# nackdai/aten

Hardware: AMD Instinct MI355X
Metric: Mrays/sec (W*H*spp/1e6/s, reference definition), Sponza 1080p 1spp 5-bounce (higher is better)
Workload: dtype f32; 1 GPU; sponza_lod 1920x1080 1spp 5-bounce GGX+IBL, reference-built sponza_lod.sbvh (stand-in for missing sponza.obj); width=1920, height=1080, spp=1, max_depth=5, rr_depth=3, frames_in_flight=4, triangles=12852, bvh_nodes=38000, anyhit_twins=1, planar_area_lights=0

## Files before the change

### aten_amd/_lib.py

```python
import ctypes as C
import os

from . import build

_lib = None

K_NAMES = ["gen_path", "trace_closest", "shade", "trace_shadow", "accumulate_sample", "gather",
           "svgf_prepare", "svgf_temporal", "svgf_variance", "svgf_atrous", "trace_fused"]

SYMBOLS = [
    "atn_create", "atn_destroy", "atn_last_error", "atn_upload_scene", "atn_update_camera", "atn_update_tlas",
    "atn_init_sampler", "atn_set_random", "atn_set_screen_shard", "atn_render", "atn_reset", "atn_set_path_batches",
    "atn_set_frames_in_flight", "atn_bank_streams", "atn_side_stream", "atn_mgpu_set_frames_in_flight", "atn_set_sampling_options", "atn_sample_texture",
    "atn_svgf_render", "atn_svgf_set_motion_depth", "atn_svgf_reset", "atn_svgf_set_atrous_iterations",
    "atn_svgf_download", "atn_svgf_output_device", "atn_svgf_set_dilate_temporal_weight", "atn_svgf_denoise", "atn_svgf_upload",
    "atn_restir_set_options", "atn_restir_render", "atn_restir_set_motion_depth", "atn_restir_reset", "atn_restir_capture",
    "atn_restir_download", "atn_npr_render", "atn_npr_reset", "atn_npr_capture", "atn_npr_download",
    "atn_volume_render", "atn_volume_reset", "atn_volume_capture", "atn_volume_download", "atn_volume_phase_table",
    "atn_ao_set_params", "atn_ao_render", "atn_ao_reset", "atn_ao_capture", "atn_ao_download",
    "atn_film_device", "atn_tile_device", "atn_tile_slots", "atn_anyhit_twins", "atn_planar_area_lights", "atn_stream", "atn_synchronize",
    "atn_assemble_tiles", "atn_assemble_tiles_on", "atn_download_film", "atn_upload_film", "atn_get_stats", "atn_get_kernel_times",
    "atn_reset_kernel_times", "atn_generate_paths", "atn_trace_closest", "atn_cmj_samples", "atn_cmj_batch", "atn_ray_offset", "atn_get_random", "atn_random_count",
    "atn_material_table", "atn_material_eval", "atn_compact", "atn_compact2", "atn_sizeof_scene_desc", "atn_sizeof_destination",
    "atn_abi_version", "atn_build_id",
    "atn_download_path_cost", "atn_update_geometry", "atn_scene_device_arrays", "atn_lbvh_rebuild_list", "atn_lbvh_build",
    "atn_mgpu_update_geometry", "atn_mgpu_lbvh_rebuild_list",
    "atn_skin_create", "atn_skin_update", "atn_skin_compute", "atn_lbvh_rebuild_list_skinned", "atn_skin_download",
    "atn_skin_download_list", "atn_skin_destroy",
    "atn_set_geometry_motion", "atn_geometry_motion_stats", "atn_geometry_motion_matrices",
    "atn_taa_resolve", "atn_taa_upload", "atn_taa_download", "atn_taa_reset", "atn_taa_output_device", "atn_taa_rgba8_device",
    "atn_mgpu_create", "atn_mgpu_destroy", "atn_mgpu_last_error", "atn_mgpu_shard_count", "atn_mgpu_shard_device",
    "atn_mgpu_upload_scene", "atn_mgpu_update_tlas", "atn_mgpu_update_camera", "atn_mgpu_init_sampler",
    "atn_mgpu_set_random", "atn_mgpu_render", "atn_mgpu_reset", "atn_mgpu_synchronize", "atn_mgpu_film_device",
    "atn_mgpu_download_film",
    "atn_set_regeneration", "atn_get_regeneration", "atn_render_burst", "atn_regen_stage_counts",
    "atn_mgpu_set_regeneration", "atn_mgpu_render_burst", "atn_set_upload_options", "atn_libm_probe", "atn_set_shade_math",
]


class Destination(C.Structure):
    _fields_ = [("width", C.c_int32), ("height", C.c_int32), ("maxDepth", C.c_int32),
                ("russianRouletteDepth", C.c_int32), ("sample", C.c_int32), ("frame", C.c_uint32),
                ("progressive", C.c_int32), ("break_on_terminate", C.c_int32),
                ("count_stats", C.c_int32), ("profile", C.c_int32)]


def lib():
    global _lib
    if _lib is None:
        path = os.environ.get("ATEN_AMD_LIB", build.HIP_LIB)
        if not os.path.exists(path):
            raise RuntimeError(
                "aten_amd: %s is missing. Build it with `python -m aten_amd.build hip` "
                "(or __graft_entry__.build()); there is no CPU fallback." % path)
        l = C.CDLL(path)
        vp = C.c_void_p
        l.atn_create.argtypes = [C.POINTER(vp), C.c_int]
        l.atn_destroy.argtypes = [vp]; l.atn_destroy.restype = None
        l.atn_last_error.argtypes = [vp]; l.atn_last_error.restype = C.c_char_p
        l.atn_upload_scene.argtypes = [vp, vp]
        l.atn_update_camera.argtypes = [vp, vp]
        l.atn_update_tlas.argtypes = [vp, vp, C.c_uint32, vp, C.c_uint32, vp, C.c_uint32]
        l.atn_download_path_cost.argtypes = [vp, vp]
        l.atn_update_geometry.argtypes = [vp, vp, vp, C.c_uint32, C.c_uint32, vp, C.c_uint32, C.c_uint32]
        l.atn_scene_device_arrays.argtypes = [vp, vp, vp, vp]
        l.atn_lbvh_rebuild_list.argtypes = [vp, C.c_uint32, C.c_uint32, C.c_uint32, vp, vp]
        l.atn_lbvh_build.argtypes = [vp, vp, C.c_uint32, C.c_int32, vp, vp, vp, C.c_uint32, C.c_int32, vp, vp, vp]
        l.atn_skin_create.argtypes = [vp, vp, C.c_uint32, C.c_uint32, C.c_uint32, C.c_uint32, C.c_uint32, C.POINTER(C.c_uint32)]
        l.atn_skin_update.argtypes = [vp, C.c_uint32, vp, C.c_uint32]
        l.atn_skin_compute.argtypes = [vp, C.c_uint32, C.c_int32, vp, vp]
        l.atn_lbvh_rebuild_list_skinned.argtypes = [vp, C.c_uint32, C.c_uint32]
        l.atn_skin_download.argtypes = [vp, C.c_uint32, C.c_int32, vp]
        l.atn_skin_download_list.argtypes = [vp, C.c_uint32, vp, C.c_uint32, C.POINTER(C.c_uint32)]
        l.atn_skin_destroy.argtypes = [vp, C.c_uint32]
        l.atn_set_geometry_motion.argtypes = [vp, C.c_int32]
        l.atn_geometry_motion_stats.argtypes = [vp, vp]
        l.atn_geometry_motion_matrices.argtypes = [vp, vp, vp]
        l.atn_mgpu_update_geometry.argtypes = [vp, vp, vp, C.c_uint32, C.c_uint32, vp, C.c_uint32, C.c_uint32]
        l.atn_mgpu_lbvh_rebuild_list.argtypes = [vp, C.c_uint32, C.c_uint32, C.c_uint32, vp, vp]
        l.atn_init_sampler.argtypes = [vp, C.c_int32, C.c_int32, C.c_int32]
        l.atn_set_random.argtypes = [vp, vp, C.c_uint32]
        l.atn_get_random.argtypes = [vp, vp, C.c_uint32]
        l.atn_random_count.argtypes = [vp]; l.atn_random_count.restype = C.c_uint32
        l.atn_set_screen_shard.argtypes = [vp, C.c_int32, C.c_int32]
        l.atn_render.argtypes = [vp, C.POINTER(Destination), vp]
        l.atn_reset.argtypes = [vp]
        l.atn_set_upload_options.argtypes = [vp, C.c_int32, C.c_int32, C.c_int32, C.c_int32]
        l.atn_set_regeneration.argtypes = [vp, C.c_int32]
        l.atn_set_shade_math.argtypes = [vp, C.c_int32]
        l.atn_get_regeneration.argtypes = [vp]; l.atn_get_regeneration.restype = C.c_int32
        l.atn_render_burst.argtypes = [vp, C.POINTER(Destination), C.c_int32, vp]
        l.atn_regen_stage_counts.argtypes = [vp, vp, vp, C.c_uint32, C.POINTER(C.c_uint32)]
        l.atn_set_path_batches.argtypes = [vp, C.c_int32]
        l.atn_set_frames_in_flight.argtypes = [vp, C.c_int32]
        l.atn_bank_streams.argtypes = [vp, C.POINTER(C.c_int32), C.POINTER(C.c_int32)]
        l.atn_set_sampling_options.argtypes = [vp, C.c_int32, C.c_int32]
        l.atn_sample_texture.argtypes = [vp, C.c_int32, C.c_uint32, vp, vp]
        l.atn_mgpu_set_frames_in_flight.argtypes = [vp, C.c_int32]
        l.atn_svgf_render.argtypes = [vp, vp, C.c_int32, vp, vp]
        l.atn_svgf_set_motion_depth.argtypes = [vp, vp, C.c_uint32]
        l.atn_svgf_reset.argtypes = [vp]
        l.atn_svgf_set_atrous_iterations.argtypes = [vp, C.c_int32]
        l.atn_svgf_download.argtypes = [vp, C.c_int32, vp]
        l.atn_restir_set_options.argtypes = [vp, C.c_int32, C.c_int32]
        l.atn_restir_render.argtypes = [vp, vp, C.c_int32, vp]
        l.atn_restir_set_motion_depth.argtypes = [vp, vp, C.c_uint32]
        l.atn_restir_reset.argtypes = [vp]
        l.atn_restir_capture.argtypes = [vp, C.c_int32]
        l.atn_restir_download.argtypes = [vp, C.c_int32, vp]
        l.atn_npr_render.argtypes = [vp, vp, vp]
        l.atn_npr_reset.argtypes = [vp]
        l.atn_npr_capture.argtypes = [vp, C.c_int32]
        l.atn_npr_download.argtypes = [vp, C.c_int32, vp]
        l.atn_volume_render.argtypes = [vp, vp, vp]
        l.atn_volume_reset.argtypes = [vp]
        l.atn_volume_capture.argtypes = [vp, C.c_int32]
        l.atn_volume_download.argtypes = [vp, C.c_int32, vp]
        l.atn_volume_phase_table.argtypes = [vp, C.c_float, C.c_uint32, vp, vp, vp, vp, vp, vp]
        l.atn_ao_set_params.argtypes = [vp, C.c_int32, C.c_float, C.c_int32]
        l.atn_ao_render.argtypes = [vp, vp, vp]
        l.atn_ao_reset.argtypes = [vp]
        l.atn_ao_capture.argtypes = [vp, C.c_int32]
        l.atn_ao_download.argtypes = [vp, C.c_int32, vp]
        l.atn_svgf_set_dilate_temporal_weight.argtypes = [vp, C.c_int32]
        l.atn_svgf_denoise.argtypes = [vp, vp, C.c_int32, vp, vp]
        l.atn_svgf_upload.argtypes = [vp, C.c_int32, C.c_int32, C.c_int32, vp]
        l.atn_svgf_output_device.argtypes = [vp]
        l.atn_svgf_output_device.restype = vp
        l.atn_taa_resolve.argtypes = [vp, C.c_int32, C.c_int32, C.c_int32, C.c_int32, C.c_float, vp, vp]
        l.atn_taa_upload.argtypes = [vp, C.c_int32, C.c_int32, C.c_int32, vp]
        l.atn_taa_download.argtypes = [vp, C.c_int32, vp]
        l.atn_taa_reset.argtypes = [vp]
        l.atn_taa_output_device.argtypes = [vp]; l.atn_taa_output_device.restype = vp
        l.atn_taa_rgba8_device.argtypes = [vp]; l.atn_taa_rgba8_device.restype = vp
        l.atn_film_device.argtypes = [vp]; l.atn_film_device.restype = vp
        l.atn_tile_device.argtypes = [vp]; l.atn_tile_device.restype = vp
        l.atn_tile_slots.argtypes = [vp]; l.atn_tile_slots.restype = C.c_uint32
        l.atn_anyhit_twins.argtypes = [vp]; l.atn_anyhit_twins.restype = C.c_uint32
        l.atn_planar_area_lights.argtypes = [vp]; l.atn_planar_area_lights.restype = C.c_uint32
        l.atn_stream.argtypes = [vp]; l.atn_stream.restype = vp
        l.atn_side_stream.argtypes = [vp]; l.atn_side_stream.restype = vp
        l.atn_synchronize.argtypes = [vp]
        l.atn_assemble_tiles.argtypes = [vp, vp, C.c_int32, vp]
        l.atn_assemble_tiles_on.argtypes = [vp, vp, C.c_int32, vp, vp]
        l.atn_download_film.argtypes = [vp, vp]
        l.atn_upload_film.argtypes = [vp, C.c_int32, C.c_int32, vp]
        l.atn_get_stats.argtypes = [vp, vp]
        l.atn_get_kernel_times.argtypes = [vp, vp, vp]
        l.atn_reset_kernel_times.argtypes = [vp]
        l.atn_generate_paths.argtypes = [vp, C.c_int32, C.c_int32, C.c_int32, C.c_uint32, vp]
        l.atn_trace_closest.argtypes = [vp, vp, C.c_uint32, C.c_float, C.c_float, vp, vp]
        l.atn_cmj_samples.argtypes = [vp, C.c_uint32, C.c_uint32, C.c_uint32, C.c_int32, vp]
        l.atn_cmj_batch.argtypes = [vp, C.c_uint32, vp, vp, vp, C.c_int32, vp]
        l.atn_ray_offset.argtypes = [vp, C.c_uint32, vp, vp, vp]
        l.atn_libm_probe.argtypes = [vp, C.c_int32, C.c_uint32, vp, vp, vp]
        l.atn_material_table.argtypes = [vp, C.c_int32, C.c_uint32, vp, vp, vp, vp, vp, vp, vp, vp]
        l.atn_material_eval.argtypes = [vp, C.c_int32, C.c_uint32, vp, vp, vp, vp, vp]
        l.atn_compact.argtypes = [vp, vp, C.c_uint32, vp, C.POINTER(C.c_uint32)]
        l.atn_compact2.argtypes = [vp, vp, vp, C.c_uint32, C.c_uint32, vp, C.POINTER(C.c_uint32), vp, C.POINTER(C.c_uint32)]
        l.atn_mgpu_create.argtypes = [C.POINTER(vp), vp, C.c_int32]
        l.atn_mgpu_destroy.argtypes = [vp]; l.atn_mgpu_destroy.restype = None
        l.atn_mgpu_last_error.argtypes = [vp]; l.atn_mgpu_last_error.restype = C.c_char_p
        l.atn_mgpu_shard_count.argtypes = [vp]; l.atn_mgpu_shard_count.restype = C.c_int32
        l.atn_mgpu_shard_device.argtypes = [vp, C.c_int32]; l.atn_mgpu_shard_device.restype = C.c_int32
        l.atn_mgpu_upload_scene.argtypes = [vp, vp]
        l.atn_mgpu_update_tlas.argtypes = [vp, vp, C.c_uint32, vp, C.c_uint32, vp, C.c_uint32]
        l.atn_mgpu_update_camera.argtypes = [vp, vp]
        l.atn_mgpu_init_sampler.argtypes = [vp, C.c_int32, C.c_int32, C.c_int32]
        l.atn_mgpu_set_random.argtypes = [vp, vp, C.c_uint32]
        l.atn_mgpu_render.argtypes = [vp, C.POINTER(Destination), vp]
        l.atn_mgpu_reset.argtypes = [vp]
        l.atn_mgpu_set_regeneration.argtypes = [vp, C.c_int32]
# ... 10 lines not shown
```

### aten_amd/csrc/aten_amd.hip

```cpp
#include <hip/hip_runtime.h>

#include <algorithm>
#include <cstdio>
#include <cstdlib>
#include <chrono>
#include <cstring>
#include <memory>
#include <random>
#include <string>
#include <vector>

#include "../../include/aten_amd.h"
#include "device/kernels.hpp"
#include "device/launch.hpp"
#include "device/svgf.hpp"
#include "device/restir.hpp"
#include "device/npr.hpp"
#include "device/ao.hpp"
#include "device/volume.hpp"
#include "device/lbvh.hpp"
#include "device/skinning.hpp"
#include "device/motion.hpp"
#include "device/taa.hpp"
#include "host/scene_upload.hpp"
#include "host/ibl_precompute.hpp"

namespace atn {

#define ATN_HIP(expr)                                                                      \
    do {                                                                                   \
        hipError_t e_ = (expr);                                                            \
        if (e_ != hipSuccess) { return fail(ATN_ERR_HIP, std::string(#expr) + ": " + hipGetErrorString(e_)); } \
    } while (0)

template <class T>
struct DevBuf {
    T* p = nullptr;
    size_t n = 0;
    ~DevBuf() { release(); }
    void release() { if (p) { (void)hipFree(p); p = nullptr; n = 0; } }
    hipError_t resize(size_t count)
    {
        if (count <= n && p) return hipSuccess;
        release();
        if (count == 0) return hipSuccess;
        hipError_t e = hipMalloc((void**)&p, count * sizeof(T) + 256);
        if (e == hipSuccess) n = count;
        return e;
    }
    void swap(DevBuf& o) { std::swap(p, o.p); std::swap(n, o.n); }
    hipError_t upload(const std::vector<T>& v, hipStream_t s)
    {
        hipError_t e = resize(v.size() ? v.size() : 1);
        if (e != hipSuccess || v.empty()) return e;
        return hipMemcpyAsync(p, v.data(), v.size() * sizeof(T), hipMemcpyHostToDevice, s);
    }
};

__global__ void k_spin(unsigned long long ticks)
{
    const unsigned long long t0 = wall_clock64();
    while (wall_clock64() - t0 < ticks) { }
}
constexpr unsigned long long kSpinTicks = 30000;
inline bool streams_run_side_by_side(hipStream_t a, hipStream_t b, bool& ok)
{
    const double spin_us = (double)kSpinTicks / 100.0;
    for (int rep = 0; rep < 3; rep++) {
        if (hipStreamSynchronize(a) != hipSuccess || hipStreamSynchronize(b) != hipSuccess) { ok = false; return false; }
        const auto t0 = std::chrono::steady_clock::now();
        hipLaunchKernelGGL(k_spin, dim3(1), dim3(1), 0, a, kSpinTicks);
        hipLaunchKernelGGL(k_spin, dim3(1), dim3(1), 0, b, kSpinTicks);
        if (hipStreamSynchronize(a) != hipSuccess || hipStreamSynchronize(b) != hipSuccess) { ok = false; return false; }
        const double us = std::chrono::duration<double, std::micro>(std::chrono::steady_clock::now() - t0).count();
        ok = true;
        if (us < 1.5 * spin_us) return true;
    }
    ok = true;
    return false;
}

class PathTracing {
public:
    std::string last_error;
    int device = 0;
    hipStream_t stream = nullptr;
    static constexpr int kMaxBatches = 8;
    static constexpr int kMaxShards = 64;
    hipStream_t bstream[kMaxBatches] = {};
    hipEvent_t ev_fork = nullptr, ev_join[kMaxBatches] = {};
    int n_batches = 3;
    bool batches_forced = false;
    bool fuse_traces = true;
    bool env_probe_streams = true;
    bool env_lds_nodes = true;
    int env_anyhit_twin = 1;
    int env_anyhit_twin_dirs = 8;
    bool opt_node_layout = true, opt_planar_lights = true;
    bool env_atrous4 = true;
    int env_shade_waves = 0;
    int env_flavour = -1;

    DevBuf<float4> nodes, vtx_pos, vtx_nml, matrices, texels, carpaint, shade_tris;
    DevBuf<atn_triangle_param> tris;
    DevBuf<atn_object_param> objects;
    DevBuf<DevMaterial> materials;
    DevBuf<atn_light_param> lights;
    DevBuf<float4> light_plane;
    DevBuf<DevTexture> textures;
    DevBuf<atn_toon_param> toon;
    DevBuf<atn_light_param> npr_lights;
    DevBuf<float> screen_shadow;
    DevBuf<uint32_t> texels8;
    DevScene scene{};
    bool has_scene = false, has_camera = false;
    std::vector<int32_t> list_root_link;
    uint32_t n_planar_lights = 0;
    struct PlanarCert {
        int32_t inst_obj = -1, mesh_obj = -1, mtx_id = -1;
        atn_object_param inst{}, mesh{};
        atn_mat4 l2w{}, w2l{};
        uint32_t tri_first = 0, tri_count = 0, vtx_lo = 0, vtx_hi = 0;
    };
    std::vector<PlanarCert> planar_certs;
    void collect_planar_certs(const atn_scene_desc* s, const std::vector<atn_light_param>& lights)
    {
        planar_certs.clear();
        for (size_t i = 0; i < lights.size() && i < s->n_lights; i++) {
            if (!lights[i]._pad) continue;
            PlanarCert c;
            c.inst_obj = s->lights[i].arealight_objid;
            c.inst = s->objects[c.inst_obj];
            const atn_object_param* o = &s->objects[c.inst_obj];
            if (o->type == ATN_OBJ_INSTANCE) {
                c.mtx_id = o->mtx_id;
                if (c.mtx_id >= 0) { c.l2w = s->matrices[c.mtx_id]; c.w2l = s->matrices[c.mtx_id + 1]; }
                c.mesh_obj = o->object_id;
                c.mesh = s->objects[c.mesh_obj];
                o = &s->objects[c.mesh_obj];
            }
            c.tri_first = (uint32_t)o->triangle_id; c.tri_count = (uint32_t)o->triangle_num;
            c.vtx_lo = 0xFFFFFFFFu; c.vtx_hi = 0;
            for (uint32_t t = c.tri_first; t < c.tri_first + c.tri_count; t++)
                for (int k = 0; k < 3; k++) {
                    const uint32_t v = (uint32_t)s->triangles[t].idx[k];
                    c.vtx_lo = std::min(c.vtx_lo, v); c.vtx_hi = std::max(c.vtx_hi, v);
                }
            planar_certs.push_back(c);
        }
    }
    bool planar_certs_survive_objects(const atn_object_param* objs, uint32_t n_objs, const atn_mat4* mtxs, uint32_t n_mtxs) const
    {
        for (const PlanarCert& c : planar_certs) {
            if ((uint32_t)c.inst_obj >= n_objs || std::memcmp(&objs[c.inst_obj], &c.inst, sizeof(atn_object_param)) != 0) return false;
            if (c.mesh_obj >= 0 && ((uint32_t)c.mesh_obj >= n_objs || std::memcmp(&objs[c.mesh_obj], &c.mesh, sizeof(atn_object_param)) != 0)) return false;
            if (c.mtx_id >= 0 && n_mtxs
                && ((uint32_t)c.mtx_id + 1 >= n_mtxs || std::memcmp(&mtxs[c.mtx_id], &c.l2w, sizeof(atn_mat4)) != 0
                    || std::memcmp(&mtxs[c.mtx_id + 1], &c.w2l, sizeof(atn_mat4)) != 0)) return false;
        }
        return true;
    }
    bool planar_certs_survive_geometry(uint32_t vtx_offset, uint32_t n_vtx, uint32_t tri_offset, uint32_t n_tr) const
    {
        for (const PlanarCert& c : planar_certs) {
            if (n_vtx && vtx_offset <= c.vtx_hi && (uint64_t)vtx_offset + n_vtx > c.vtx_lo) return false;
            if (n_tr && tri_offset < c.tri_first + c.tri_count && (uint64_t)tri_offset + n_tr > c.tri_first) return false;
        }
        return true;
    }
    std::vector<int32_t> list_twin_delta;
    std::vector<HostSceneImage::TlasRef> tlas_refs;
    uint32_t top_base = 0, n_host_matrices = 0;
    std::vector<atn_mat4> host_matrices;
    std::vector<uint32_t> list_base, list_bytes, list_tri_leaves, list_inner;
    uint32_t n_scene_tris = 0, n_scene_vtx = 0, n_scene_mtrls = 0;

    struct LbvhScratch {
        DevBuf<uint32_t> codes[2], indices[2], counts, totals, arrived, offs;
        DevBuf<uint8_t> flips;
        DevBuf<int32_t> left, right, parent, first, last;
        DevBuf<atn_bvh_node> ref_nodes;
        DevBuf<LbvhBox> pre, suf, sup;
        DevBuf<atn_triangle_param> tris;
// ... 393 lines not shown
        t->tick = cur_tick;
        cur_tick = ++tick_counter;
        point_scene_at_current_set();
        return ATN_OK;
    }

    hipEvent_t ev_scene = nullptr, ev_stage = nullptr;
    hipStream_t scene_stream = nullptr;
    hipStream_t upd = nullptr;
    uint64_t scene_epoch = 0, bank_epoch = 0;
    bool stage_busy = false;
    char* stage_p = nullptr;
    size_t stage_cap = 0, stage_used = 0;

    int begin_scene_update(size_t stage_bytes)
    {
        if (!ev_scene) { ATN_HIP(hipEventCreateWithFlags(&ev_scene, hipEventDisableTiming)); ATN_HIP(hipEventCreateWithFlags(&ev_stage, hipEventDisableTiming)); }
        if (stage_busy) { ATN_HIP(hipEventSynchronize(ev_stage)); stage_busy = false; }
        stage_used = 0;
        if (stage_bytes > stage_cap) {
            if (stage_p) ATN_HIP(hipHostFree(stage_p));
            stage_p = nullptr; stage_cap = 0;
            const size_t cap = stage_bytes + stage_bytes / 2 + 4096;
            ATN_HIP(hipHostMalloc((void**)&stage_p, cap, hipHostMallocDefault));
            stage_cap = cap;
        }
        if (frames_in_flight > 1 && !scene_stream) ATN_HIP(hipStreamCreateWithFlags(&scene_stream, hipStreamNonBlocking));
        upd = frames_in_flight > 1 ? scene_stream : stream;
        if (frames_in_flight > 1 && n_spare_ready > 0 && !scene_in_place) {
            if (frame_since_update) { int r = flip_scene_set(); if (r) return r; frame_since_update = false; }
            return ATN_OK;
        }
        if (n_alt > 0 && frames_in_flight <= 1) drop_alt_set();
        log_now.clear();
        if (upd != stream) {
            for (int i = 0; i < n_spare_ready; i++) if (spare[i].ev_gather) ATN_HIP(hipStreamWaitEvent(upd, spare[i].ev_gather, 0));
            if (ev_gather) ATN_HIP(hipStreamWaitEvent(upd, ev_gather, 0));
        }
        return ATN_OK;
    }
    int stage_copy(void* dst_dev, const void* src_host, size_t bytes)
    {
        if (!bytes) return ATN_OK;
        const size_t off = (stage_used + 63) & ~(size_t)63;
        if (off + bytes > stage_cap) return fail(ATN_ERR_INVALID_ARG, "staging arena too small (internal)");
        std::memcpy(stage_p + off, src_host, bytes);
        stage_used = off + bytes;
        ATN_HIP(hipMemcpyAsync(dst_dev, stage_p + off, bytes, hipMemcpyHostToDevice, upd));
        return ATN_OK;
    }
    int end_scene_update()
    {
        if (stage_used) { ATN_HIP(hipEventRecord(ev_stage, upd)); stage_busy = true; }
        ATN_HIP(hipEventRecord(ev_scene, upd));
        scene_epoch++;
        if (upd == stream) bank_epoch = scene_epoch;
        return ATN_OK;
    }
    int record_scene_read()
    {
        ATN_HIP(hipEventRecord(ev_gather, stream));
        hipEvent_t& e = ev_read[bank_scene_set];
        if (!e) ATN_HIP(hipEventCreateWithFlags(&e, hipEventDisableTiming));
        ATN_HIP(hipEventRecord(e, stream));
        return ATN_OK;
    }
    int wait_scene_epoch()
    {
        if (bank_epoch != scene_epoch && ev_scene) ATN_HIP(hipStreamWaitEvent(stream, ev_scene, 0));
        bank_epoch = scene_epoch;
        bank_scene_set = cur_set;
        frame_since_update = true;
        return ATN_OK;
    }

    float k_ms[ATN_K_COUNT] = {};
    uint32_t k_launches[ATN_K_COUNT] = {};
    std::vector<hipEvent_t> ev_pool;
    struct Span { int kind; size_t e0, e1; };
    static constexpr size_t kMaxSpans = 8192;
    std::vector<Span> spans;
    size_t ev_used = 0;
    hipStream_t prof_stream = nullptr;
    uint64_t host_stats[8] = {};

    int fail(int code, const std::string& msg) { last_error = msg; return code; }

    int init(int device_ordinal)
    {
        int n = 0;
        hipError_t e = hipGetDeviceCount(&n);
        if (e != hipSuccess || n <= 0) return fail(ATN_ERR_NO_DEVICE, "no HIP device available (libaten_amd has no CPU fallback)");
        if (device_ordinal < 0 || device_ordinal >= n) return fail(ATN_ERR_INVALID_ARG, "device ordinal out of range");
        device = device_ordinal;
        ATN_HIP(hipSetDevice(device));
        ATN_HIP(hipStreamCreateWithFlags(&stream, hipStreamNonBlocking));
        for (int k = 0; k < kMaxBatches; k++) {
            ATN_HIP(hipStreamCreateWithFlags(&bstream[k], hipStreamNonBlocking));
            ATN_HIP(hipEventCreateWithFlags(&ev_join[k], hipEventDisableTiming));
        }
        ATN_HIP(hipEventCreateWithFlags(&ev_fork, hipEventDisableTiming));
        ATN_HIP(hipEventCreateWithFlags(&ev_gather, hipEventDisableTiming));
        if (const char* e = std::getenv("ATEN_AMD_FUSE")) fuse_traces = e[0] != '0';
        if (const char* e = std::getenv("ATEN_AMD_SVGF_ATROUS4")) env_atrous4 = e[0] != '0';
        if (const char* e = std::getenv("ATEN_AMD_SHADE_WAVES")) { const int v = std::atoi(e); if (v == 4 || v == 5) env_shade_waves = v; }
        if (const char* e = std::getenv("ATEN_AMD_LDS_NODES")) env_lds_nodes = std::atoi(e) != 0;
        if (const char* e = std::getenv("ATEN_AMD_ANYHIT_TWIN")) env_anyhit_twin = std::max(0, std::min(2, std::atoi(e)));
        if (const char* e = std::getenv("ATEN_AMD_ANYHIT_TWIN_DIRS")) env_anyhit_twin_dirs = std::atoi(e) == 1 ? 1 : 8;
        if (const char* e = std::getenv("ATEN_AMD_NODE_LAYOUT")) opt_node_layout = std::atoi(e) != 0;
        if (const char* e = std::getenv("ATEN_AMD_PLANAR_LIGHTS")) opt_planar_lights = std::atoi(e) != 0;
        if (const char* e = std::getenv("ATEN_AMD_PROBE_STREAMS")) env_probe_streams = std::atoi(e) != 0;
        if (const char* e = std::getenv("ATEN_AMD_TRACE")) { env_flavour = e[0] == 'r' ? 1 : 0; }
        if (const char* e = std::getenv("ATEN_AMD_BATCHES")) {
            n_batches = std::atoi(e);
            batches_forced = true;
            if (n_batches < 1) n_batches = 1;
            if (n_batches > kMaxBatches) n_batches = kMaxBatches;
        }
        return ATN_OK;
    }

    ~PathTracing()
    {
        for (auto& e : ev_pool) (void)hipEventDestroy(e);
        for (int k = 0; k < kMaxBatches; k++) {
            if (ev_join[k]) (void)hipEventDestroy(ev_join[k]);
            if (bstream[k]) (void)hipStreamDestroy(bstream[k]);
        }
        if (ev_fork) (void)hipEventDestroy(ev_fork);
        if (rs_ev) (void)hipEventDestroy(rs_ev);
        if (ta_ev) (void)hipEventDestroy(ta_ev);
        if (gm_ev) (void)hipEventDestroy(gm_ev);
        if (ao_ev) (void)hipEventDestroy(ao_ev);
        if (ev_gather) (void)hipEventDestroy(ev_gather);
        for (auto& e : sv_ev_prepare) if (e) (void)hipEventDestroy(e);
        if (ev_film) (void)hipEventDestroy(ev_film);
        if (sv_stream) (void)hipStreamDestroy(sv_stream);
        for (int i = 0; i < n_spare_ready; i++) {
            Bank& b = spare[i];
            for (int k = 0; k < kMaxBatches; k++) {
                if (b.ev_join[k]) (void)hipEventDestroy(b.ev_join[k]);
                if (b.bstream[k]) (void)hipStreamDestroy(b.bstream[k]);
            }
            if (b.ev_fork) (void)hipEventDestroy(b.ev_fork);
            if (b.ev_gather) (void)hipEventDestroy(b.ev_gather);
            for (auto& e : b.ev_read) if (e) (void)hipEventDestroy(e);
            if (b.stream) (void)hipStreamDestroy(b.stream);
        }
        if (stream) (void)hipStreamDestroy(stream);
        if (side_stream) (void)hipStreamDestroy(side_stream);
        if (scene_stream) (void)hipStreamDestroy(scene_stream);
        for (auto& e : ev_read) if (e) (void)hipEventDestroy(e);
        if (ev_scene) (void)hipEventDestroy(ev_scene);
        if (ev_stage) (void)hipEventDestroy(ev_stage);
        if (stage_p) (void)hipHostFree(stage_p);
    }

    int UpdateSceneData(const atn_scene_desc* s)
    {
        ATN_HIP(hipSetDevice(device));
        { int q = quiesce(); if (q) return q; }
        drop_alt_set(); cur_set = 0; scene_in_place = false; frame_since_update = true;
        skins.clear();
        HostSceneImage img;
        std::string err;
        const int layout_top = opt_node_layout ? kLayoutTopLevels : 0;
        const bool planar_lights = opt_planar_lights;
        if (!build_host_image(img, s, err, env_anyhit_twin, env_anyhit_twin_dirs, layout_top, planar_lights)) return fail(ATN_ERR_UNSUPPORTED, err);
        n_planar_lights = 0;
        for (const atn_light_param& l : img.lights) n_planar_lights += l._pad != 0 ? 1u : 0u;
        collect_planar_certs(s, img.lights);
        ATN_HIP(nodes.upload(img.nodes, stream));
        ATN_HIP(tris.upload(img.tris, stream));
        ATN_HIP(vtx_pos.upload(img.vtx_pos, stream));
        ATN_HIP(vtx_nml.upload(img.vtx_nml, stream));
        ATN_HIP(objects.upload(img.objects, stream));
        ATN_HIP(matrices.upload(img.matrices, stream));
        ATN_HIP(materials.upload(img.materials, stream));
        ATN_HIP(carpaint.upload(img.carpaint, stream));
        ATN_HIP(toon.upload(img.toon, stream));
        ATN_HIP(npr_lights.upload(img.npr_lights, stream));
        ATN_HIP(screen_shadow.upload(img.screen_shadow, stream));
        ATN_HIP(lights.upload(img.lights, stream));
        ATN_HIP(light_plane.upload(img.light_plane, stream));
        ATN_HIP(texels.upload(img.texels, stream));
        ATN_HIP(texels8.upload(img.texels8, stream));
        ATN_HIP(textures.upload(img.textures, stream));
        ATN_HIP(shade_tris.resize((size_t)kShadeTriQuads * (img.tris.size() ? img.tris.size() : 1)));
        if (!img.tris.empty())
// ... 472 lines not shown
    {
        if (!has_scene) return fail(ATN_ERR_NO_SCENE, "atn_upload_scene has not been called");
        if (list == 0 || list >= list_base.size()) return fail(ATN_ERR_INVALID_ARG, "not a bottom-level BVH list");
        const int32_t twin_word = list < list_twin_delta.size() ? list_twin_delta[list] : 0;
        const uint32_t twin_delta = (uint32_t)(twin_word & ~15), twin_dirs = twin_word == 0 ? 0u : ((twin_word & 1) ? 8u : 1u);
        const uint64_t bytes = twin_dirs ? (uint64_t)twin_delta * (1u + twin_dirs) : list_bytes[list];
        if ((uint64_t)list_base[list] + bytes > nodes.n * sizeof(float4)) return fail(ATN_ERR_UNSUPPORTED, "the list's region leaves the node image (internal)");
        if (n_bytes) *n_bytes = (uint32_t)bytes;
        if (!out) return ATN_OK;
        if (capacity < bytes) return fail(ATN_ERR_INVALID_ARG, "output buffer too small for the list");
        ATN_HIP(hipSetDevice(device));
        { int q = quiesce(); if (q) return q; }
        ATN_HIP(hipMemcpyAsync(out, reinterpret_cast<char*>(nodes.p) + list_base[list], bytes, hipMemcpyDeviceToHost, stream));
        ATN_HIP(hipStreamSynchronize(stream));
        return ATN_OK;
    }

    int updateCamera(const atn_camera_param* c)
    {
        if (!c) return fail(ATN_ERR_INVALID_ARG, "null camera");
        camera = *c;
        has_camera = true;
        return ATN_OK;
    }

    int setRandom(const uint32_t* v, uint32_t n)
    {
        if (!v || n == 0) return fail(ATN_ERR_INVALID_ARG, "empty seed array");
        ATN_HIP(hipSetDevice(device));
        { int q = quiesce(); if (q) return q; }
        ATN_HIP(seeds.resize(n));
        ATN_HIP(hipMemcpyAsync(seeds.p, v, (size_t)n * 4, hipMemcpyHostToDevice, stream));
        ATN_HIP(hipStreamSynchronize(stream));
        n_seeds = n;
        return ATN_OK;
    }

    int getRandom(uint32_t* out, uint32_t n)
    {
        if (!out || n == 0 || n > n_seeds) return fail(ATN_ERR_INVALID_ARG, "atn_get_random: null output or more entries than the sampler holds");
        ATN_HIP(hipSetDevice(device));
        { int q = quiesce(); if (q) return q; }
        ATN_HIP(hipMemcpyAsync(out, seeds.p, (size_t)n * 4, hipMemcpyDeviceToHost, stream));
        ATN_HIP(hipStreamSynchronize(stream));
        return ATN_OK;
    }

    int initSampler(int32_t w, int32_t h, int32_t seed)
    {
        if (w <= 0 || h <= 0) return fail(ATN_ERR_INVALID_ARG, "bad sampler size");
        std::vector<uint32_t> v((size_t)w * h);
        std::mt19937 src(seed);
        for (auto& x : v) x = (uint32_t)src();
        return setRandom(v.data(), (uint32_t)v.size());
    }

    int ensure_frame(int32_t w, int32_t h, int32_t max_depth)
    {
        const int32_t tx = (w + 7) / 8, ty = (h + 7) / 8;
        const uint32_t n_tiles = (uint32_t)tx * ty;
        const uint32_t tiles_per_rank = (n_tiles + world - 1) / world;
        const uint32_t slots = tiles_per_rank * 64;
        if (slots > kShadowSlotMask) return fail(ATN_ERR_UNSUPPORTED, "more than 2^26 path slots per GPU (shard the screen)");
        if (slots != n_slots) {
            ATN_HIP(ray_o.resize(slots)); ATN_HIP(ray_d.resize(slots)); ATN_HIP(thr.resize(slots));
            ATN_HIP(contrib.resize(slots)); ATN_HIP(isect.resize(slots));
            ATN_HIP(sh_o.resize(slots)); ATN_HIP(sh_d.resize(slots)); ATN_HIP(sh_c.resize(slots));
            ATN_HIP(accum.resize(slots)); ATN_HIP(done.resize(slots));
            ATN_HIP(queue0.resize(slots)); ATN_HIP(queue1.resize(slots)); ATN_HIP(shadow_q.resize(slots));
            ATN_HIP(tile_out.resize(slots));
            n_slots = slots;
        }
        if (w != film_w || h != film_h) {
            if (frames_in_flight > 1) { int qrc = quiesce(); if (qrc) return qrc; }
            ATN_HIP(film.resize((size_t)w * h));
            ATN_HIP(hipMemsetAsync(film.p, 0, (size_t)w * h * sizeof(float4), stream));
            film_w = w; film_h = h;
        }
        if (max_depth + 2 > counters_depth) {
            ATN_HIP(counters.resize((size_t)kMaxBatches * 4 * (max_depth + 2)));
            counters_depth = max_depth + 2;
        }
        if (!stats.p) {
            ATN_HIP(stats.resize(8));
            ATN_HIP(hipMemsetAsync(stats.p, 0, 64, stream));
        }
        return ATN_OK;
    }

    PathBuffers buffers(bool count, int batch = 0, uint32_t slot_begin = 0)
    {
        PathBuffers pb{};
        pb.ray_o = ray_o.p; pb.ray_d = ray_d.p; pb.thr = thr.p; pb.contrib = contrib.p; pb.seeds = seeds.p;
        pb.isect = isect.p; pb.sh_o = sh_o.p; pb.sh_d = sh_d.p; pb.sh_c = sh_c.p;
        pb.accum = accum.p; pb.done = done.p; pb.queue[0] = queue0.p + slot_begin; pb.queue[1] = queue1.p + slot_begin;
        pb.shadow_q = shadow_q.p + slot_begin;
        uint32_t* cb = counters.p + (size_t)batch * 4 * counters_depth;
        pb.q_count = cb; pb.sh_count = cb + counters_depth;
        pb.fetch_closest = cb + 2 * counters_depth; pb.fetch_shadow = cb + 3 * counters_depth;
        pb.stats = count ? stats.p : nullptr;
        pb.cost = count ? cost.p : nullptr;
        return pb;
    }

    FrameParams frame_params(const atn_destination& d)
    {
        FrameParams fp{};
        fp.width = d.width; fp.height = d.height; fp.n_slots = (int32_t)n_slots;
        fp.tiles_x = (d.width + 7) / 8; fp.tiles_y = (d.height + 7) / 8; fp.tiles_x_rcp = udiv_rcp((uint32_t)fp.tiles_x);
        fp.rank = rank; fp.world = world;
        fp.max_depth = d.maxDepth;
        fp.rr_depth = d.russianRouletteDepth;
        if (fp.rr_depth > fp.max_depth) fp.rr_depth = fp.max_depth - 1;
        fp.slot_begin = 0; fp.slot_end = (int32_t)n_slots;
        fp.chunk_items = kChunkItems;
        fp.sample = 0; fp.frame = d.frame; fp.n_seeds = n_seeds;
        fp.break_on_terminate = d.break_on_terminate; fp.progressive = d.progressive;
        return fp;
    }

    static uint32_t grid_for(uint32_t n, uint32_t cap_blocks = 256u * 16u)
    {
        uint32_t b = (n + 255u) / 256u;
        if (b == 0) b = 1;
        return b < cap_blocks ? b : cap_blocks;
    }

    bool tree_is_deep = false;
    static constexpr size_t kRefillMinNodes = 2048;
    static constexpr uint32_t kRefillMinPaths = 400u * 1000u;
    bool refill_walk(bool frame) const
    {
        if (env_flavour >= 0) return env_flavour == 1;
        return tree_is_deep && (!frame || n_slots >= kRefillMinPaths);
    }

    uint32_t lds_scene_bytes() const
    {
        const uint64_t b = (uint64_t)scene.node_bytes + (uint64_t)scene.mtx_quads * 16u;
        return (env_lds_nodes && b <= kLdsNodesMaxBytes) ? (uint32_t)b : 0u;
    }

    uint32_t trace_grid(uint32_t n_jobs, bool refill) const
    {
        if (refill) {
            const uint32_t waves_per_block = (uint32_t)kTraceBlock / 64u;
            uint32_t blocks = ((n_jobs + atn::kFetchChunk - 1u) / atn::kFetchChunk + waves_per_block - 1u) / waves_per_block;
            if (blocks < 1u) blocks = 1u;
            const uint32_t cap = (frames_in_flight > 1 ? 256u * 18u : 256u * 32u) / waves_per_block;
            return blocks < cap ? blocks : cap;
        }
        return grid_for(n_jobs);
    }

    PassPlan plan_pass(PassKind kind, uint32_t n) const
    {
        PassPlan p{};
        p.kind = kind;
        p.refill = refill_walk(true);
        p.lds_bytes = lds_scene_bytes();
        p.block = p.lds_bytes > 8192u ? 256u : 64u;
        p.trace_grid = trace_grid(n, p.refill);
        p.fused_grid = trace_grid(2u * n, p.refill);
        p.shade_items = n >= 400u * 1000u ? kChunkItems : 2;
        p.shade_grid = grid_for((n + (uint32_t)p.shade_items - 1u) / (uint32_t)p.shade_items);
        const bool big = n >= 1500u * 1000u;
        p.shade_waves = env_shade_waves ? env_shade_waves
                      : (kind == PassKind::Serial && frames_in_flight > 1 && (scene.material_set != kMsCore || big) ? 5 : 4);
        return p;
    }

    template <bool SHADOW>
    void launch_trace(const PassPlan& p, const PathBuffers& pb, bool count, int32_t b, hipStream_t st)
    {
        const dim3 g(p.trace_grid), t(p.refill ? (uint32_t)kTraceBlock : 256u);
        with_flags([&](auto c, auto refill) {
            if constexpr (SHADOW) hipLaunchKernelGGL((k_trace_shadow<decltype(c)::value, decltype(refill)::value>), g, t, 0, st, pb, scene, b);
            else hipLaunchKernelGGL((k_trace_closest<decltype(c)::value, decltype(refill)::value>), g, t, 0, st, pb, scene, b);
        }, count, p.refill);
    }

    template <bool SVGF>
    void launch_shade(const PassPlan& p, hipStream_t st, const PathBuffers& pb, const FrameParams& fp, int32_t b, const SvgfShade& sv)
    {
        if (!SVGF && shade_math_relaxed) {
            relaxed_launch_shade(scene.material_set, p.shade_waves, p.shade_grid, st, pb, scene, fp, camera, b);
            return;
        }
        with_shade_flavour(scene.material_set, p.shade_waves, [&](auto k) {
            using K = decltype(k);
            if constexpr (K::waves == 0) hipLaunchKernelGGL((k_shade<SVGF, K::ms>), dim3(p.shade_grid), dim3(256), 0, st, pb, scene, fp, camera, b, sv);
            else hipLaunchKernelGGL((k_shade_wn<SVGF, K::ms, K::waves>), dim3(p.shade_grid), dim3(256), 0, st, pb, scene, fp, camera, b, sv);
        });
    }

    void prof_begin(bool on, int kind, hipStream_t st = nullptr)
    {
        if (!st) st = stream;
        prof_stream = st;
        if (!on) return;
        if (spans.size() >= kMaxSpans) {
            (void)hipStreamSynchronize(stream);
            for (int k = 0; k < kMaxBatches; k++) (void)hipStreamSynchronize(bstream[k]);
            prof_collect();
        }
        if (ev_used + 2 > ev_pool.size()) {
            for (int i = 0; i < 64; i++) { hipEvent_t e; (void)hipEventCreate(&e); ev_pool.push_back(e); }
        }
        spans.push_back(Span{ kind, ev_used, ev_used + 1 });
        (void)hipEventRecord(ev_pool[ev_used], st);
    }
    void prof_end(bool on)
    {
        if (!on) return;
        (void)hipEventRecord(ev_pool[ev_used + 1], prof_stream);
        ev_used += 2;
    }
    void prof_collect()
    {
        for (const Span& s : spans) {
            float ms = 0;
            if (hipEventElapsedTime(&ms, ev_pool[s.e0], ev_pool[s.e1]) == hipSuccess) { k_ms[s.kind] += ms; k_launches[s.kind]++; }
        }
        spans.clear();
        ev_used = 0;
    }

    template <bool SVGF>
    int run_paths(const atn_destination* d, FrameParams fp, bool count, bool prof, const SvgfShade& sv, const SvgfFrame& sf)
    {
        int nb;
        if (batches_forced) {
            nb = n_batches;
            const uint32_t min_batch = 200u * 1000u;
            while (nb > 1 && n_slots / (uint32_t)nb < min_batch) nb--;
        }
        else {
            nb = refill_walk(true) ? 1 : (lds_scene_bytes() && frames_in_flight > 1) ? 1 : (n_slots >= (frames_in_flight > 1 ? 1500u : 800u) * 1000u ? 2 : 1);
            if (nb > n_batches) nb = n_batches;
        }
        if (nb > batch_streams_checked && nb > 1 && env_probe_streams) { int rc = separate_batch_streams(nb); if (rc) return rc; }
        uint32_t per = (n_slots + (uint32_t)nb - 1u) / (uint32_t)nb;
        per = (per + kChunk - 1u) / kChunk * kChunk;
        ATN_HIP(hipMemsetAsync(counters.p, 0, (size_t)nb * 4 * counters_depth * 4, stream));
        ATN_HIP(hipEventRecord(ev_fork, stream));
        for (int k = 0; k < nb; k++) {
            const uint32_t begin = (uint32_t)k * per;
            const uint32_t end = begin + per < n_slots ? begin + per : n_slots;
            if (begin >= end) continue;
            hipStream_t st = nb > 1 ? bstream[k] : stream;
            if (nb > 1) ATN_HIP(hipStreamWaitEvent(st, ev_fork, 0));
            PathBuffers pb = buffers(count, k, begin);
            fp.slot_begin = (int32_t)begin; fp.slot_end = (int32_t)end;
            const uint32_t n = end - begin;
            const PassPlan plan = plan_pass(SVGF ? PassKind::Svgf : PassKind::Serial, n);
            fp.chunk_items = plan.shade_items;
            const uint32_t g_slots = grid_for(n), g_all = (n + 255u) / 256u;
            for (int32_t s = 0; s < d->sample; s++) {
                fp.sample = s;
                if (s > 0) ATN_HIP(hipMemsetAsync(pb.q_count, 0, (size_t)4 * counters_depth * 4, st));
                prof_begin(prof, ATN_K_GEN, st);
                hipLaunchKernelGGL(k_gen_path, dim3(g_slots), dim3(256), 0, st, pb, fp, camera, (const uint32_t*)seeds.p);
                prof_end(prof);
                if (count || !fuse_traces) {
                    for (int32_t b = 0; b < d->maxDepth; b++) {
                        prof_begin(prof, ATN_K_TRACE_CLOSEST, st);
                        launch_trace<false>(plan, pb, count, b, st);
                        prof_end(prof);
                        if (SVGF && b == 0 && gm_capture) motion_launch_capture(g_all, st, pb, fp, gm_capture);
                        prof_begin(prof, ATN_K_SHADE, st);
                        launch_shade<SVGF>(plan, st, pb, fp, b, sv);
                        prof_end(prof);
                        prof_begin(prof, ATN_K_TRACE_SHADOW, st);
                        launch_trace<true>(plan, pb, count, b, st);
                        prof_end(prof);
                    }
                }
                else {
                    for (int32_t b = 0; b <= d->maxDepth; b++) {
                        const TraceLaunch tl = trace_launch(plan, b);
                        prof_begin(prof, tl.prof_kind, st);
                        launch_trace_fused<false>(tl, st, pb, scene, b - 1, b < d->maxDepth ? b : -1, b);
                        prof_end(prof);
                        if (SVGF && b == 0 && gm_capture) motion_launch_capture(g_all, st, pb, fp, gm_capture);
                        if (b < d->maxDepth) {
                            prof_begin(prof, ATN_K_SHADE, st);
                            launch_shade<SVGF>(plan, st, pb, fp, b, sv);
                            prof_end(prof);
                        }
                    }
                }
                if (SVGF || d->sample > 1) {
                    prof_begin(prof, ATN_K_ACCUM, st);
                    if (SVGF) hipLaunchKernelGGL(k_svgf_sample_end, dim3(g_all), dim3(256), 0, st, pb, fp, sf);
                    else hipLaunchKernelGGL(k_accumulate_sample, dim3(g_all), dim3(256), 0, st, pb, fp);
                    prof_end(prof);
                }
            }
            if (nb > 1) {
                ATN_HIP(hipEventRecord(ev_join[k], st));
                ATN_HIP(hipStreamWaitEvent(stream, ev_join[k], 0));
            }
        }
        return ATN_OK;
    }

    int check_ready(const atn_destination* d)
    {
        if (!d) return fail(ATN_ERR_INVALID_ARG, "null destination");
        if (!has_scene) return fail(ATN_ERR_NO_SCENE, "atn_upload_scene has not been called");
        if (!has_camera) return fail(ATN_ERR_INVALID_ARG, "atn_update_camera has not been called");
        if (n_seeds == 0) return fail(ATN_ERR_INVALID_ARG, "atn_init_sampler / atn_set_random has not been called");
        if (d->width <= 0 || d->height <= 0 || d->maxDepth <= 0 || d->sample <= 0) return fail(ATN_ERR_INVALID_ARG, "bad destination");
        return ATN_OK;
    }
    int begin_frame(const atn_destination& d, bool rotate)
    {
        if (rotate) swap_bank(spare[frame_seq % (uint64_t)(frames_in_flight - 1)]);
        frame_seq++;
        const int rc = wait_scene_epoch();
        return rc ? rc : ensure_frame(d.width, d.height, d.maxDepth);
    }
    int wait_film()
    {
        if (film_pending) ATN_HIP(hipStreamWaitEvent(stream, ev_film, 0));
        return taa_before_write(stream);
    }
    int record_film_writer()
    {
        if (frames_in_flight <= 1) return ATN_OK;
        if (!ev_film) ATN_HIP(hipEventCreateWithFlags(&ev_film, hipEventDisableTiming));
        ATN_HIP(hipEventRecord(ev_film, stream));
        film_pending = true;
        return ATN_OK;
    }
    int end_film_frame()
    {
        const int rc = frames_in_flight > 1 ? record_scene_read() : ATN_OK;
        return rc ? rc : record_film_writer();
    }

    int render(const atn_destination* d, atn_vec4* out_host)
    {
        int rc = check_ready(d);
        if (rc) return rc;
        ATN_HIP(hipSetDevice(device));
        if (d->sample > 1 && regen_applies(*d, 1)) return render_regen(d, 1, out_host);
        const bool count = d->count_stats != 0, prof = d->profile != 0;
        if (frames_in_flight > 1 && count) { rc = quiesce(); if (rc) return rc; }
        rc = begin_frame(*d, frames_in_flight > 1 && !count);
        if (rc) return rc;
        FrameParams fp = frame_params(*d);
        if (count) {
            ATN_HIP(hipMemsetAsync(stats.p, 0, 64, stream));
            ATN_HIP(cost.resize((size_t)2 * n_slots));
            ATN_HIP(cost_film.resize((size_t)2 * d->width * d->height));
            ATN_HIP(hipMemsetAsync(cost.p, 0, (size_t)2 * n_slots * sizeof(uint32_t), stream));
            ATN_HIP(hipMemsetAsync(cost_film.p, 0, (size_t)2 * d->width * d->height * sizeof(uint32_t), stream));
            cost_w = d->width; cost_h = d->height;
        }
        PathBuffers pb = buffers(count);

        const uint32_t g_all = (n_slots + 255u) / 256u;
        rc = run_paths<false>(d, fp, count, prof, SvgfShade{}, SvgfFrame{});
        if (rc) return rc;
        fp.slot_begin = 0; fp.slot_end = (int32_t)n_slots;
        rc = wait_film();
        if (rc) return rc;
        prof_begin(prof, ATN_K_GATHER);
        if (d->sample == 1) hipLaunchKernelGGL((k_gather<true>), dim3(g_all), dim3(256), 0, stream, pb, fp, film.p, tile_out.p);
        else hipLaunchKernelGGL((k_gather<false>), dim3(g_all), dim3(256), 0, stream, pb, fp, film.p, tile_out.p);
        prof_end(prof);
        ATN_HIP(hipGetLastError());
        rc = end_film_frame();
        if (rc) return rc;

        if (count) {
            hipLaunchKernelGGL(k_cost_to_pixels, dim3(g_all), dim3(256), 0, stream, fp, (const uint32_t*)cost.p, cost_film.p);
            ATN_HIP(hipMemcpyAsync(host_stats, stats.p, 64, hipMemcpyDeviceToHost, stream));
        }
        if (out_host) {
            ATN_HIP(hipMemcpyAsync(out_host, film.p, (size_t)d->width * d->height * sizeof(float4), hipMemcpyDeviceToHost, stream));
        }
        if (out_host || count) ATN_HIP(hipStreamSynchronize(stream));
        return ATN_OK;
    }


    bool shade_math_relaxed = false;
    int regen_mode = 0;
    uint64_t rg_host_totals[4] = {};
    static constexpr int32_t kRegenMaxStages = 1 << 16;
    static constexpr int32_t kRegenMaxDepth = 128;
    static constexpr size_t kRegenStagingBytes = (size_t)1 << 30;

    bool regen_applies(const atn_destination& d, int32_t n_frames) const
    {
        if (regen_mode == 0 || d.count_stats) return false;
        if (d.maxDepth > kRegenMaxDepth || (uint32_t)d.sample >= kRegenMaxSpp) return false;
        if ((uint64_t)n_frames * (uint64_t)d.width * (uint64_t)d.height >= kRegenMaxItems) return false;
        if (n_frames > 1 && !d.progressive) return false;
        return ((int64_t)n_frames + 1) * d.sample * d.maxDepth <= kRegenMaxStages;
    }

    int render_burst(const atn_destination* d, int32_t n_frames, atn_vec4* out_host)
    {
        if (!d) return fail(ATN_ERR_INVALID_ARG, "null destination");
        if (n_frames <= 0) return fail(ATN_ERR_INVALID_ARG, "bad burst length");
        if (regen_applies(*d, n_frames)) {
            { const int rc = check_ready(d); if (rc) return rc; }
            ATN_HIP(hipSetDevice(device));
            const uint64_t tiles = (uint64_t)((d->width + 7) / 8) * ((d->height + 7) / 8);
            const uint64_t plane = ((tiles + world - 1) / world) * 64u * sizeof(float4);
            int32_t piece = (int32_t)(kRegenStagingBytes / (plane ? plane : 1u));
            if (piece < 1) piece = 1;
            atn_destination part = *d;
            for (int32_t k = 0; k < n_frames; k += piece) {
                const int32_t n = n_frames - k < piece ? n_frames - k : piece;
                part.frame = d->frame + (uint32_t)k;
                const int rc = render_regen(&part, n, k + n == n_frames ? out_host : nullptr);
                if (rc) return rc;
            }
            return ATN_OK;
        }
        atn_destination one = *d;
        for (int32_t k = 0; k < n_frames; k++) {
            one.frame = d->frame + (uint32_t)k;
            const int rc = render(&one, k + 1 == n_frames ? out_host : nullptr);
            if (rc) return rc;
        }
        return ATN_OK;
    }

    int render_regen(const atn_destination* d, int32_t n_frames, atn_vec4* out_host)
    {
        const bool prof = d->profile != 0;
        int rc = begin_frame(*d, frames_in_flight > 1);
        if (rc) return rc;
        const int32_t stages = (n_frames + 1) * d->sample * d->maxDepth;
        rc = regen_valid_list(d->width, d->height);
        if (rc) return rc;
        if (pend.n < n_slots) ATN_HIP(pend.resize(n_slots));
        const size_t cstride = (size_t)stages + 3;
        if (rg_counters.n < 3 * cstride + 1) ATN_HIP(rg_counters.resize(3 * cstride + 1));
        if (rg_frames.n < (size_t)n_frames * n_slots) ATN_HIP(rg_frames.resize((size_t)n_frames * n_slots));
        rg_stages = stages;
        FrameParams fp = frame_params(*d);
        fp.burst_frames = n_frames; fp.spp = d->sample;
        fp.n_valid = rg_n_valid; fp.n_valid_rcp = udiv_rcp(rg_n_valid); fp.n_items = rg_n_valid * (uint32_t)n_frames;
        PathBuffers pb = buffers(false);
        pb.pend = pend.p;
        pb.valid_list = rg_valid.p; pb.next_item = rg_counters.p + 3 * cstride;
        pb.q_count = rg_counters.p + 1; pb.sh_count = rg_counters.p + cstride + 1; pb.fetch_closest = rg_counters.p + 2 * cstride + 1;
        pb.fetch_shadow = nullptr;
        const RegenOut ro{ rg_frames.p, film.p, tile_out.p };

        const uint32_t n = rg_n_valid;
        const PassPlan plan = plan_pass(PassKind::Regen, n);
        fp.chunk_items = plan.shade_items;
        const uint32_t g_all = (n_slots + 255u) / 256u;
        const uint32_t chunk_size = 256u * (uint32_t)plan.shade_items, n_chunks = (n + chunk_size - 1u) / chunk_size, n_groups = (n_chunks + kRegenGroup - 1u) / kRegenGroup;
        const size_t region_words = (size_t)n_chunks * chunk_size;
        const size_t rg_words = 2 * region_words + 2 * (size_t)n_chunks + 4 * (size_t)n_groups;
        if (rg_regions.n < rg_words) ATN_HIP(rg_regions.resize(rg_words));
        pb.q_regions = rg_regions.p; pb.sh_regions = rg_regions.p + region_words; pb.region_counts = rg_regions.p + 2 * region_words;
        uint32_t* const group_counts[2] = { pb.region_counts + 2 * (size_t)n_chunks, pb.region_counts + 2 * (size_t)n_chunks + 2 * (size_t)n_groups };

// ... 1322 lines not shown
    CTX_OR_FAIL(ctx);
    return guarded(ctx, [&] { return ctx->r.skin_update(skin, matrices, n); });
}
int atn_skin_compute(atn_ctx* ctx, atn_skin skin, int32_t is_restart, float* bbox_min, float* bbox_max)
{
    CTX_OR_FAIL(ctx);
    return guarded(ctx, [&] { return ctx->r.skin_compute(skin, is_restart != 0, bbox_min, bbox_max); });
}
int atn_lbvh_rebuild_list_skinned(atn_ctx* ctx, uint32_t list_index, atn_skin skin)
{
    CTX_OR_FAIL(ctx);
    return guarded(ctx, [&] { return ctx->r.lbvh_rebuild_list_skinned(list_index, skin); });
}
int atn_skin_download(atn_ctx* ctx, atn_skin skin, int32_t which, void* out_host)
{
    CTX_OR_FAIL(ctx);
    return guarded(ctx, [&] { return ctx->r.skin_download(skin, which, out_host); });
}
int atn_skin_download_list(atn_ctx* ctx, uint32_t list_index, void* out_host, uint32_t capacity_bytes, uint32_t* n_bytes)
{
    CTX_OR_FAIL(ctx);
    return guarded(ctx, [&] { return ctx->r.download_list(list_index, out_host, capacity_bytes, n_bytes); });
}
int atn_skin_destroy(atn_ctx* ctx, atn_skin skin)
{
    CTX_OR_FAIL(ctx);
    return guarded(ctx, [&] { return ctx->r.skin_destroy(skin); });
}
int atn_scene_device_arrays(atn_ctx* ctx, void** vtx_pos, void** vtx_nml, void** triangles)
{
    CTX_QUIET_OR_FAIL(ctx);
    if (!ctx->r.has_scene) return ctx->r.fail(ATN_ERR_NO_SCENE, "atn_upload_scene has not been called");
    { int q = ctx->r.quiesce(); if (q) return q; }
    ctx->r.drop_alt_set(); ctx->r.scene_in_place = true;
    if (ctx->r.gm_on) { const int g = ctx->r.set_geometry_motion(0); if (g) return g; }
    ctx->r.scene.planar_lights = 0;
    if (vtx_pos) *vtx_pos = ctx->r.vtx_pos.p;
    if (vtx_nml) *vtx_nml = ctx->r.vtx_nml.p;
    if (triangles) *triangles = ctx->r.tris.p;
    return ATN_OK;
}
int atn_set_geometry_motion(atn_ctx* ctx, int32_t on)
{
    CTX_QUIET_OR_FAIL(ctx);
    return guarded(ctx, [&] { return ctx->r.set_geometry_motion(on); });
}
int atn_geometry_motion_stats(atn_ctx* ctx, uint64_t* out3)
{
    CTX_OR_FAIL(ctx);
    if (!out3) return ctx->r.fail(ATN_ERR_INVALID_ARG, "null output");
    for (int k = 0; k < 3; k++) out3[k] = ctx->r.gm_stats[k];
    return ATN_OK;
}
int atn_geometry_motion_matrices(atn_ctx* ctx, float* w2c16, float* prev_w2c16)
{
    CTX_OR_FAIL(ctx);
    if (!w2c16 || !prev_w2c16) return ctx->r.fail(ATN_ERR_INVALID_ARG, "null output");
    if (!ctx->r.gm_stats[0]) return ctx->r.fail(ATN_ERR_INVALID_ARG, "no frame has been rendered with compute_motion = 2");
    std::memcpy(w2c16, ctx->r.gm_w2c, sizeof(ctx->r.gm_w2c)); std::memcpy(prev_w2c16, ctx->r.gm_prev_w2c, sizeof(ctx->r.gm_prev_w2c));
    return ATN_OK;
}
int atn_init_sampler(atn_ctx* ctx, int32_t w, int32_t h, int32_t seed) { CTX_QUIET_OR_FAIL(ctx); return guarded(ctx, [&] { return ctx->r.initSampler(w, h, seed); }); }
int atn_get_random(atn_ctx* ctx, uint32_t* out_host, uint32_t n) { CTX_QUIET_OR_FAIL(ctx); return guarded(ctx, [&] { return ctx->r.getRandom(out_host, n); }); }
uint32_t atn_random_count(atn_ctx* ctx) { return ctx ? ctx->r.n_seeds : 0; }
int atn_set_random(atn_ctx* ctx, const uint32_t* seeds, uint32_t n) { CTX_QUIET_OR_FAIL(ctx); return guarded(ctx, [&] { return ctx->r.setRandom(seeds, n); }); }

int atn_set_screen_shard(atn_ctx* ctx, int32_t rank, int32_t world)
{
    CTX_OR_FAIL(ctx);
    if (world <= 0 || rank < 0 || rank >= world) return ctx->r.fail(ATN_ERR_INVALID_ARG, "bad screen shard");
    ctx->r.rank = rank; ctx->r.world = world;
    return ATN_OK;
}

int atn_render(atn_ctx* ctx, const atn_destination* dst, atn_vec4* out_host) { CTX_OR_FAIL(ctx); return guarded(ctx, [&] { return ctx->r.render(dst, out_host); }); }
int atn_render_burst(atn_ctx* ctx, const atn_destination* dst, int32_t n_frames, atn_vec4* out_host) { CTX_OR_FAIL(ctx); return guarded(ctx, [&] { return ctx->r.render_burst(dst, n_frames, out_host); }); }
int atn_set_regeneration(atn_ctx* ctx, int32_t mode)
{
    CTX_QUIET_OR_FAIL(ctx);
    if (mode < 0 || mode > 1) return ctx->r.fail(ATN_ERR_INVALID_ARG, "regeneration mode out of range");
    ctx->r.regen_mode = mode;
    return ATN_OK;
}
int atn_set_shade_math(atn_ctx* ctx, int32_t mode)
{
    CTX_QUIET_OR_FAIL(ctx);
    if (mode < 0 || mode > 1) return ctx->r.fail(ATN_ERR_INVALID_ARG, "shade math mode out of range");
    ctx->r.shade_math_relaxed = mode == 1;
    return ATN_OK;
}
int32_t atn_get_regeneration(atn_ctx* ctx) { return ctx ? ctx->r.regen_mode : 0; }
int atn_regen_stage_counts(atn_ctx* ctx, uint32_t* closest, uint32_t* shadow, uint32_t capacity, uint32_t* n_stages)
{
    CTX_QUIET_OR_FAIL(ctx);
    return guarded(ctx, [&] { return ctx->r.regen_stage_counts(closest, shadow, capacity, n_stages); });
}
int atn_reset(atn_ctx* ctx) { CTX_QUIET_OR_FAIL(ctx); return ctx->r.reset(); }
int atn_set_path_batches(atn_ctx* ctx, int32_t n)
{
    CTX_OR_FAIL(ctx);
    if (n < 1 || n > PathTracing::kMaxBatches) return ctx->r.fail(ATN_ERR_INVALID_ARG, "batch count out of range");
    ctx->r.n_batches = n;
    ctx->r.batches_forced = n == 1;
    return ATN_OK;
}

int atn_set_sampling_options(atn_ctx* ctx, int32_t ibl_importance, int32_t tex_bilinear)
{
    CTX_OR_FAIL(ctx);
    return guarded(ctx, [&] { return ctx->r.set_sampling_options(ibl_importance, tex_bilinear); });
}

int atn_sample_texture(atn_ctx* ctx, int32_t texid, uint32_t n, const float* uv_host, float* out_host)
{
    CTX_QUIET_OR_FAIL(ctx);
    PathTracing& r = ctx->r;
    if (!r.has_scene) return r.fail(ATN_ERR_NO_SCENE, "atn_upload_scene has not been called");
    if (texid < 0 || texid >= r.scene.n_textures || n == 0 || !uv_host || !out_host) return r.fail(ATN_ERR_INVALID_ARG, "bad texture id / count");
    return guarded(ctx, [&]() -> int {
        C_HIP(r, hipSetDevice(r.device));
        atn::DevBuf<float> duv, dout;
        C_HIP(r, duv.resize(2 * (size_t)n)); C_HIP(r, dout.resize(4 * (size_t)n));
        C_HIP(r, hipMemcpyAsync(duv.p, uv_host, 8 * (size_t)n, hipMemcpyHostToDevice, r.stream));
        hipLaunchKernelGGL(atn::k_sample_texture, dim3((n + 255) / 256), dim3(256), 0, r.stream, r.scene, texid, n, (const float*)duv.p, dout.p);
        C_HIP(r, hipGetLastError());
        C_HIP(r, hipMemcpyAsync(out_host, dout.p, 16 * (size_t)n, hipMemcpyDeviceToHost, r.stream));
        C_HIP(r, hipStreamSynchronize(r.stream));
        return ATN_OK;
    });
}

int atn_set_frames_in_flight(atn_ctx* ctx, int32_t n)
{
    CTX_OR_FAIL(ctx);
    return guarded(ctx, [&] { return ctx->r.set_frames_in_flight(n); });
}

int atn_bank_streams(atn_ctx* ctx, int32_t* swaps, int32_t* concurrent)
{
    CTX_OR_FAIL(ctx);
    return guarded(ctx, [&] {
        atn::PathTracing& r = ctx->r;
        C_HIP(r, hipSetDevice(r.device));
        { int q = r.quiesce(); if (q) return q; }
        if (swaps) *swaps = r.n_stream_swaps;
        if (concurrent) {
            *concurrent = 1;
            hipStream_t st[atn::PathTracing::kMaxInFlight];
            st[0] = r.stream;
            for (int i = 1; i < r.frames_in_flight; i++) st[i] = r.spare[i - 1].stream;
            for (int i = 0; i < r.frames_in_flight; i++)
                for (int j = 0; j < i; j++) {
                    bool ok = true;
                    if (!atn::streams_run_side_by_side(st[j], st[i], ok)) *concurrent &= ~1;
                    if (!ok) return r.fail(ATN_ERR_HIP, "stream probe failed");
                }
            if (r.side_stream) {
                *concurrent |= 2;
                for (int i = 0; i < r.frames_in_flight; i++) {
                    bool ok = true;
                    if (!atn::streams_run_side_by_side(st[i], r.side_stream, ok)) *concurrent &= ~2;
                    if (!ok) return r.fail(ATN_ERR_HIP, "stream probe failed");
                }
            }
        }
        return (int)ATN_OK;
// ... 571 lines not shown
```

### aten_amd/csrc/device/kernels.hpp

```cpp
#pragma once
#include "shading.hpp"
#include "toon.hpp"

#if defined(ATN_REGEN_TU) || defined(ATN_TEMPLATES_ONLY)
#define ATN_MAIN_TU 0
#else
#define ATN_MAIN_TU 1
#endif
#ifdef ATN_REGEN_TU
#define ATN_REGEN_KERNELS 1
#else
#define ATN_REGEN_KERNELS 0
#endif

namespace atn {

constexpr uint32_t F_TERMINATED = 1u, F_SINGULAR = 2u, F_HIT = 4u;
constexpr uint32_t kShadowSlotMask = (1u << 26) - 1u;
constexpr uint32_t kShadowStencilFlag = 0x40000000u;
constexpr uint32_t F_LAST_SPECULAR = 8u;

constexpr uint32_t F_PENDING = 16u;
constexpr uint32_t kRegenFlagMask = 31u;
constexpr uint32_t kRegenBounceShift = 5u, kRegenBounceMask = 255u;
constexpr uint32_t kRegenSampleShift = 13u, kRegenSampleMask = 2047u;
constexpr uint32_t kRegenItemHiShift = 24u;
constexpr uint32_t kRegenDimMask = 4095u, kRegenItemLoShift = 12u, kRegenItemLoMask = (1u << 20) - 1u;
constexpr uint32_t kRegenMaxSpp = 1u << 11, kRegenMaxItems = 1u << 28;
constexpr uint32_t kShadowFinalFlag = 0x20000000u;

struct PathBuffers {
    float4* ray_o;
    float4* ray_d;
    float4* thr;
    float4* contrib;
    const uint32_t* seeds;
    float4* isect;
    float4* sh_o;
    float4* sh_d;
    float4* sh_c;
    float4* accum;
    uint32_t* done;
    uint32_t* queue[2];
    uint32_t* shadow_q;
    uint32_t* q_count;
    uint32_t* sh_count;
    uint32_t* fetch_closest;
    uint32_t* fetch_shadow;
    uint32_t* cost;
    unsigned long long* stats;
    float4* pend;
    uint32_t* q_regions;
    uint32_t* sh_regions;
    uint32_t* region_counts;
    uint32_t* group_counts;
    const uint32_t* valid_list;
    uint32_t* next_item;
};

struct FrameParams {
    int32_t width, height;
    int32_t n_slots;
    int32_t slot_begin, slot_end;
    int32_t chunk_items;
    int32_t tiles_x, tiles_y;
    uint32_t tiles_x_rcp;
    int32_t rank, world;
    int32_t max_depth, rr_depth;
    int32_t sample;
    uint32_t frame;
    uint32_t n_seeds;
    int32_t break_on_terminate;
    int32_t progressive;
    int32_t burst_frames, spp;
    uint32_t n_valid, n_valid_rcp, n_items;
};

ATN_DEV bool slot_to_pixel(const FrameParams& fp, uint32_t slot, int32_t& x, int32_t& y)
{
    const uint32_t local_tile = slot >> 6;
    const uint32_t in_tile = slot & 63u;
    const uint32_t tile = local_tile * (uint32_t)fp.world + (uint32_t)fp.rank;
    if (tile >= (uint32_t)(fp.tiles_x * fp.tiles_y)) return false;
    uint32_t tx, ty;
    udivmod(tile, (uint32_t)fp.tiles_x, fp.tiles_x_rcp, ty, tx);
    x = (int32_t)tx * 8 + (int32_t)(in_tile & 7u);
    y = (int32_t)ty * 8 + (int32_t)(in_tile >> 3);
    return x < fp.width && y < fp.height;
}

constexpr int kChunkItems = 4;
constexpr uint32_t kChunk = 256u * kChunkItems;

struct BlockAppendShared { uint32_t wave_total[2][4]; uint32_t base[2]; };

template <class EntryFn, bool REGION = false>
ATN_DEV void block_append2(BlockAppendShared& sh, uint32_t* qA, uint32_t* cntA, uint32_t flagsA,
                           uint32_t* qB, uint32_t* cntB, uint32_t flagsB, EntryFn entry)
{
    const uint32_t tid = here_v(threadIdx.x);
    const uint32_t lane = tid & 63u, wave = tid >> 6;
    uint32_t totA = 0, totB = 0;
#pragma unroll
    for (int k = 0; k < kChunkItems; k++) {
        totA += (uint32_t)__popcll(__ballot((flagsA >> k) & 1u));
        totB += (uint32_t)__popcll(__ballot((flagsB >> k) & 1u));
    }
    if (lane == 0) { sh.wave_total[0][wave] = totA; sh.wave_total[1][wave] = totB; }
    __syncthreads();
    if (threadIdx.x == 0) {
        const uint32_t a = sh.wave_total[0][0] + sh.wave_total[0][1] + sh.wave_total[0][2] + sh.wave_total[0][3];
        const uint32_t b = sh.wave_total[1][0] + sh.wave_total[1][1] + sh.wave_total[1][2] + sh.wave_total[1][3];
        if constexpr (REGION) { *cntA = a; *cntB = b; sh.base[0] = 0u; sh.base[1] = 0u; }
        else {
        sh.base[0] = a ? atomicAdd(cntA, a) : 0u;
        sh.base[1] = (b && cntB) ? atomicAdd(cntB, b) : 0u;
        }
    }
    __syncthreads();
    uint32_t offA = sh.base[0], offB = sh.base[1];
    for (uint32_t w = 0; w < wave; w++) { offA += sh.wave_total[0][w]; offB += sh.wave_total[1][w]; }
#pragma unroll
    for (int k = 0; k < kChunkItems; k++) {
        const unsigned long long mA = __ballot((flagsA >> k) & 1u);
        const unsigned long long mB = __ballot((flagsB >> k) & 1u);
        if ((flagsA >> k) & 1u) qA[offA + bits_below_lane(mA)] = entry(k);
        if ((flagsB >> k) & 1u) qB[offB + bits_below_lane(mB)] = entry(k);
        offA += (uint32_t)__popcll(mA);
        offB += (uint32_t)__popcll(mB);
    }
    __syncthreads();
}

ATN_DEV void wave_add_stat(unsigned long long* dst, uint32_t v)
{
    for (int off = 32; off > 0; off >>= 1) v += __shfl_down(v, off);
    if (__lane_id() == 0 && v) atomicAdd(dst, (unsigned long long)v);
}

ATN_DEV void pinhole_sample(const atn_camera_param& cam, float s, float t, f3& org, f3& dir)
// ... 140 lines not shown
__global__ void __launch_bounds__(256) k_regen_compact(PathBuffers pb, int32_t stage, uint32_t chunk_size, uint32_t* group_counts_next, uint32_t n_groups)
{
    __shared__ uint32_t red[2][4];
    const uint32_t n_prev = pb.q_count[stage - 1];
    const uint32_t n_chunks = (n_prev + chunk_size - 1u) / chunk_size;
    const uint32_t c = blockIdx.x;
    if (c == 0u) { for (uint32_t g = threadIdx.x; g < 2u * n_groups; g += 256u) group_counts_next[g] = 0u; }
    if (c >= n_chunks) return;
    const uint32_t g0 = c / kRegenGroup;
    uint32_t sq = 0, ss = 0;
    for (uint32_t g = threadIdx.x; g < g0; g += 256u) { sq += pb.group_counts[2u * g]; ss += pb.group_counts[2u * g + 1u]; }
    for (uint32_t r = g0 * kRegenGroup + threadIdx.x; r < c; r += 256u) { sq += pb.region_counts[2u * r]; ss += pb.region_counts[2u * r + 1u]; }
    for (int off = 32; off > 0; off >>= 1) { sq += __shfl_down(sq, off); ss += __shfl_down(ss, off); }
    if ((threadIdx.x & 63u) == 0u) { red[0][threadIdx.x >> 6] = sq; red[1][threadIdx.x >> 6] = ss; }
    __syncthreads();
    const uint32_t base_q = red[0][0] + red[0][1] + red[0][2] + red[0][3];
    const uint32_t base_s = red[1][0] + red[1][1] + red[1][2] + red[1][3];
    const uint32_t nq = pb.region_counts[2u * c], ns = pb.region_counts[2u * c + 1u];
    uint32_t* __restrict__ qd = pb.queue[stage & 1];
    for (uint32_t e = threadIdx.x; e < nq; e += 256u) qd[base_q + e] = pb.q_regions[(size_t)c * chunk_size + e];
    for (uint32_t e = threadIdx.x; e < ns; e += 256u) pb.shadow_q[base_s + e] = pb.sh_regions[(size_t)c * chunk_size + e];
    if (c == n_chunks - 1u && threadIdx.x == 0u) { pb.q_count[stage] = base_q + nq; pb.sh_count[stage - 1] = base_s + ns; }
}

__global__ void __launch_bounds__(256) k_regen_flush(PathBuffers pb, FrameParams fp, RegenOut ro)
{
    const uint32_t slot = blockIdx.x * blockDim.x + threadIdx.x;
    if (slot >= (fp.n_valid < fp.n_items ? fp.n_valid : fp.n_items)) return;
    const uint32_t w = __float_as_uint(pb.ray_d[slot].w);
    if (w & F_PENDING) {
        const float4 pd = pb.pend[slot];
        regen_epilogue(pb, fp, ro, slot, mk3(pd), (uint32_t)fp.spp - 1u, __float_as_uint(pd.w), true);
    }
}

__global__ void __launch_bounds__(256) k_regen_end(PathBuffers pb, FrameParams fp, RegenOut ro)
{
    const uint32_t slot = blockIdx.x * blockDim.x + threadIdx.x;
    if (slot >= (uint32_t)fp.n_slots) return;
    int32_t x, y;
    if (!slot_to_pixel(fp, slot, x, y)) {
        if (ro.tile_out) ro.tile_out[slot] = make_float4(0.0F, 0.0F, 0.0F, 0.0F);
        return;
    }
    const uint32_t pixel = (uint32_t)(y * fp.width + x);
    float4 out = make_float4(0.0F, 0.0F, 0.0F, 0.0F);
    if (fp.progressive) out = ro.film[pixel];
    for (int32_t k = 0; k < fp.burst_frames; k++) {
        const float4 v = ro.frames[(size_t)k * (uint32_t)fp.n_slots + slot];
        if (fp.progressive) {
            const float4 cur = out;
            const float n = (float)((int32_t)cur.w);
            const float d = n + 1;
            out = make_float4((n * cur.x + v.x) / d, (n * cur.y + v.y) / d, (n * cur.z + v.z) / d, n + 1);
        }
        else {
            out = v;
        }
    }
    ro.film[pixel] = out;
    if (ro.tile_out) ro.tile_out[slot] = out;
}
#endif

#ifdef ATN_TRACE_WPE
#define ATN_TRACE_ATTR __attribute__((amdgpu_waves_per_eu(ATN_TRACE_WPE, ATN_TRACE_WPE)))
#else
#define ATN_TRACE_ATTR
#endif

template <bool COUNT, bool REFILL, class Job, bool LDSN = false>
ATN_DEV void trace_dispatch(const DevScene& sc, uint32_t count, uint32_t* fetch_counter, const Job& job, TravCounters* tc)
{
    if constexpr (REFILL) {
        __shared__ TraceShared sh;
        if (LDSN) lds_scene_copy(sc);
        trace_refill<COUNT, Job, LDSN>(sc, sh, count, fetch_counter, job, tc);
    }
    else {
        trace_simple<COUNT, Job, LDSN>(sc, count, job, tc);
    }
}

struct ClosestJob {
    PathBuffers pb;
    const uint32_t* __restrict__ q;
    float t_min;
    ATN_DEV void fetch(uint32_t j, float4& a, float4& b, float& stop_t) const { fetch_slot(q[j], a, b, stop_t); }
    ATN_DEV void fetch_slot(uint32_t slot, float4& a, float4& b, float& stop_t) const
    {
        const float4 ro = pb.ray_o[slot], rd = pb.ray_d[slot];
        stop_t = -kInf;
        a = make_float4(ro.x, ro.y, ro.z, kInf);
        b = make_float4(rd.x, rd.y, rd.z, __uint_as_float(slot));
    }
    ATN_DEV bool finish(uint32_t slot, const Hit& h, bool, float4&, float4&, float&) const
    {
        pb.isect[slot] = make_float4(__int_as_float(h.objid), h.a, h.b, __int_as_float(h.tri));
        return false;
    }
    ATN_DEV void cost(uint32_t slot, uint32_t nodes, uint32_t tris) const
    {
        if (pb.cost) { atomicAdd(&pb.cost[2u * slot], nodes); atomicAdd(&pb.cost[2u * slot + 1u], tris); }
    }
};

template <bool COUNT, bool REFILL>
__global__ void __launch_bounds__(kTraceBlock > 256 ? kTraceBlock : 256) k_trace_closest(PathBuffers pb, DevScene sc, int32_t bounce)
{
    const uint32_t count = pb.q_count[bounce];
    const ClosestJob job{ pb, pb.queue[bounce & 1], kEps };
    TravCounters tc{};
    trace_dispatch<COUNT, REFILL>(sc, count, &pb.fetch_closest[bounce], job, &tc);
    if (COUNT) {
        if (blockIdx.x == 0 && threadIdx.x == 0) atomicAdd(&pb.stats[0], (unsigned long long)count);
        wave_add_stat(&pb.stats[3], tc.nodes);
        wave_add_stat(&pb.stats[4], tc.tris);
    }
}

struct SvgfShade {
    float4* nd;
    float4* am;
    float4* primary;
    float w2c3[4];
};

#ifdef ATN_SHADE_WPE
#define ATN_SHADE_ATTR __attribute__((amdgpu_waves_per_eu(ATN_SHADE_WPE, ATN_SHADE_WPE)))
#else
#define ATN_SHADE_ATTR
#endif
#ifndef ATN_SHADE_PARTITION
#define ATN_SHADE_PARTITION 1
#endif
struct ShadePartShared { uint32_t perm[kChunk]; uint32_t wcount[kChunkItems][4][2]; };
template <bool ON> struct ShadeOrderShared { uint16_t inv[ON ? kChunk : 1]; uint8_t oflag[ON ? kChunk : 1]; };

template <bool SVGF, int MS, bool REGEN = false>
ATN_DEV void shade_body(const PathBuffers& pb, const DevScene& sc, const FrameParams& fp, const atn_camera_param& cam, int32_t bounce_arg, const SvgfShade& sv,
                        const RegenOut& ro = RegenOut{})
{
    __shared__ BlockAppendShared sh;
#if ATN_SHADE_PARTITION
    __shared__ ShadePartShared part;
    __shared__ ShadeOrderShared<REGEN> order[1];
#endif
    const uint32_t count = pb.q_count[bounce_arg];
    const uint32_t* __restrict__ q = pb.queue[bounce_arg & 1];
    uint32_t* __restrict__ qn = pb.queue[(bounce_arg + 1) & 1];
#if !ATN_SHADE_PARTITION
    uint32_t nhits = 0;
#endif

    const int items = fp.chunk_items;
    const uint32_t chunk_size = 256u * (uint32_t)items;
    for (uint32_t chunk = blockIdx.x * chunk_size; chunk < count; chunk += gridDim.x * chunk_size) {
      uint32_t push_bits = 0;
#if ATN_SHADE_PARTITION
      const uint32_t n_valid = count - chunk < chunk_size ? count - chunk : chunk_size;
      {
          const uint32_t tid = here_v(threadIdx.x);
          const uint32_t lane = tid & 63u, wave = tid >> 6;
          uint32_t hitmask = 0;
          __syncthreads();
#pragma unroll 1
          for (int k = 0; k < items; k++) {
              const uint32_t j = chunk + (uint32_t)k * 256u + threadIdx.x;
              const bool valid = j < count;
              const bool hit = valid && __float_as_int(pb.isect[q[j]].x) >= 0;
              if (hit) hitmask |= 1u << k;
              const unsigned long long bh = __ballot(hit), bm = __ballot(valid && !hit);
              if (lane == 0) { part.wcount[k][wave][0] = (uint32_t)__popcll(bh); part.wcount[k][wave][1] = (uint32_t)__popcll(bm); }
          }
          if (pb.stats) wave_add_stat(&pb.stats[2], (uint32_t)__popc(hitmask));
          __syncthreads();
          uint32_t total_hits = 0;
          for (int k = 0; k < items; k++) for (uint32_t w = 0; w < 4; w++) total_hits += part.wcount[k][w][0];
          uint32_t before_h = 0, before_m = 0;
#pragma unroll 1
          for (int k = 0; k < items; k++) {
              const uint32_t j = chunk + (uint32_t)k * 256u + threadIdx.x;
              const bool valid = j < count;
              const bool hit = (hitmask >> k) & 1u;
              const unsigned long long bh = __ballot(hit), bm = __ballot(valid && !hit);
              uint32_t bh_w = before_h, bm_w = before_m;
              for (uint32_t w = 0; w < 4; w++) {
                  if (w < wave) { bh_w += part.wcount[k][w][0]; bm_w += part.wcount[k][w][1]; }
                  before_h += part.wcount[k][w][0]; before_m += part.wcount[k][w][1];
              }
              if (valid) {
                  const uint32_t pos = hit ? bh_w + bits_below_lane(bh) : total_hits + bm_w + bits_below_lane(bm);
                  part.perm[pos] = q[j];
                  if constexpr (REGEN) order[0].inv[pos] = (uint16_t)(j - chunk);
              }
          }
          __syncthreads();
      }
#endif
#pragma unroll 1
      for (int k = 0; k < items; k++) {
#if ATN_SHADE_PARTITION
        const uint32_t e = (uint32_t)k * 256u + threadIdx.x;
        const bool valid = e < n_valid;
#else
        const uint32_t j = chunk + (uint32_t)k * 256u + threadIdx.x;
        const bool valid = j < count;
#endif
        bool push_next = false, push_shadow = false;
        uint32_t rg_need_bits = 0u;
        uint32_t slot = 0;

        if (valid) {
#if ATN_SHADE_PARTITION
            slot = part.perm[e];
#else
            slot = q[j];
#endif
            const float4 ro4 = pb.ray_o[slot], rd4 = pb.ray_d[slot];
            const f3 ray_org = mk3(ro4), ray_dir = mk3(rd4);
            float pdfb = ro4.w;
            uint32_t flags = __float_as_uint(rd4.w);
            uint32_t rg_sample = 0u, rg_item = 0u;
            int32_t bounce = bounce_arg;
            if constexpr (REGEN) {
                rg_sample = (flags >> kRegenSampleShift) & kRegenSampleMask;
                rg_item = (flags >> kRegenItemHiShift) << 20;
                bounce = (int32_t)((flags >> kRegenBounceShift) & kRegenBounceMask);
                flags &= kRegenFlagMask;
            }
            const float4 is4 = pb.isect[slot];
            const int32_t hit_objid = __float_as_int(is4.x);
            const float4 thr4 = pb.thr[slot];
            f3 throughput = mk3(thr4);
            bool wrote_ray = false, thr_stored = false;
            f3 contrib_add = mk3(0.0F);
            bool contrib_changed = false;
            uint4 s4;
            uint32_t pixel_slot = slot;
            {
                uint32_t fs = fp.frame + (uint32_t)fp.sample;
                s4.y = __float_as_uint(thr4.w);
                if constexpr (REGEN) {
                    rg_item |= s4.y >> kRegenItemLoShift;
                    s4.y &= kRegenDimMask;
                    uint32_t rg_frame;
                    regen_item(pb, fp, rg_item, rg_frame, pixel_slot);
                    fs = fp.frame + rg_frame + rg_sample;
                }
                int32_t px = 0, py = 0;
                slot_to_pixel(fp, pixel_slot, px, py);
                s4.w = (uint32_t)(py * fp.width + px);
                const uint32_t rnd = pb.seeds[s4.w < fp.n_seeds ? s4.w : s4.w % here(fp.n_seeds)];
                s4.x = fs % 256u;
                s4.z = rnd * 0x1fe3434fu * ((fs + 133u * rnd) / 256u);
            }
            Cmj smp; smp.idx = s4.x; smp.dim = s4.y; smp.scramble = s4.z;
            if constexpr (REGEN) {
                if (flags & F_PENDING) {
                    flags &= ~F_PENDING;
                    const bool prev_last = rg_sample == 0u;
                    const float4 pd = pb.pend[slot];
                    regen_epilogue(pb, fp, ro, slot, mk3(pd), prev_last ? (uint32_t)fp.spp - 1u : rg_sample - 1u, __float_as_uint(pd.w), prev_last);
                }
            }
            bool rg_stored = false;
            uint32_t rg_end = 0u;
            auto regen_end = [&](bool out_of_depth) -> uint32_t {
                f3 ctot = mk3(pb.contrib[slot]);
                if (contrib_changed) ctot = ctot + contrib_add;
                const bool pending = out_of_depth;
                const bool item_last = rg_sample + 1u >= (uint32_t)fp.spp || (fp.break_on_terminate && !out_of_depth && !regen_invalid_color(ctot));
                if (pending) pb.pend[slot] = make_float4(ctot.x, ctot.y, ctot.z, __uint_as_float(rg_item));
                else regen_epilogue(pb, fp, ro, slot, ctot, rg_sample, rg_item, item_last);
                if (item_last) return pending ? 12u : 4u;
                const RegenState st = regen_primary_state(pb, fp, cam, rg_item, rg_sample + 1u, pending ? F_PENDING : 0u);
                pb.ray_o[slot] = st.o; pb.ray_d[slot] = st.d; pb.thr[slot] = st.t;
                pb.contrib[slot] = make_float4(0.0F, 0.0F, 0.0F, 0.0F);
                return 1u;
            };

            flags &= ~F_HIT;
            const bool is_hit = hit_objid >= 0;

            if (!is_hit) {
                if (!(flags & F_TERMINATED)) {
                    f3 dir = ray_dir;
                    if (bounce == 0) {
                        int32_t ix = 0, iy = 0;
                        slot_to_pixel(fp, pixel_slot, ix, iy);
                        const float s = (float)ix / (float)here(fp.width);
                        const float t = (float)iy / (float)here(fp.height);
                        f3 o;
                        pinhole_sample(cam, s, t, o, dir);
                    }
                    const float4 emit = background_sample(sc, dir);
                    float misW = 1.0f;
                    if (SVGF && (bounce == 0 || (bounce == 1 && (flags & F_SINGULAR)))) {
                        sv.nd[s4.w] = make_float4(0.0F, 0.0F, 0.0F, -1.0F);
                        sv.am[s4.w] = make_float4(emit.x, emit.y, emit.z, -1.0F);
                        if (bounce == 0) sv.primary[s4.w] = make_float4(0.0F, 0.0F, 0.0F, 0.0F);
                    }
                    if (!(bounce == 0 || (bounce == 1 && (flags & F_SINGULAR)))) {
                        float pdfLight = luminance(emit.x, emit.y, emit.z) / sc.avgIllum;
                        pdfLight /= (2.0f * kPi);
// ... 78 lines not shown
                    shaded_out = true;
                }

                if (!shaded_out) {
                    if (!(m.attrib & ATN_MTRL_ATTR_TRANSLUCENT) && isBackfacing) orienting_normal = -orienting_normal;
                    const int32_t mtrl_slot = mtrlid >= 0 ? mtrlid : sc.n_materials;
                    const float pre_r = apply_normal<MS>(sc, m, mtrl_slot, orienting_normal, rec.u, rec.v, ray_dir, smp);

                    const bool invalid_mtrl = (m.attrib & (ATN_MTRL_ATTR_SINGULAR | ATN_MTRL_ATTR_TRANSLUCENT)) != 0;
                    const bool nee = sc.n_lights > 0 && !invalid_mtrl;
                    const uint32_t nee_dim = smp.dim;
                    const f3 thr_in = throughput;
                    HitPre hp;
                    tangent_coordinate(orienting_normal, hp.t, hp.b);
                    hp.rough = ggx_roughness(sc, m, rec.u, rec.v);
                    hp.lambda_v = m.type == ATN_MTRL_GGX ? ggx_lambda(hp.rough, -ray_dir, orienting_normal) : 0.0F;
                    int32_t nee_light = 0;
                    if (nee) {
                        if (here(sc.n_lights) > 1) {
                            nee_light = (int32_t)(cmj_next(smp) * (float)here(sc.n_lights));
                            nee_light = nee_light < sc.n_lights - 1 ? nee_light : sc.n_lights - 1;
                        }
                        else smp.dim++;
                        smp.dim += light_sample_draws(sc.lights[nee_light], sc);
                    }

                    float russian_prob = 1.0f;
                    if (bounce > fp.rr_depth) {
                        if (dot(throughput, throughput) > 0) {
                            russian_prob = max3(throughput);
                            const float p = cmj_next(smp);
                            if (p >= russian_prob) flags |= F_TERMINATED; else flags &= ~F_TERMINATED;
                        }
                    }

                    MtrlSample ms;
                    sample_material<MS>(ms, sc, m, orienting_normal, ray_dir, smp, rec.u, rec.v, mtrl_slot, pre_r, &hp);
                    const f3 next_dir = normalize(ms.dir);
                    const f3 ray_along_normal = dot(orienting_normal, next_dir) >= 0.0f ? orienting_normal : -orienting_normal;
                    const float c = dot(ray_along_normal, next_dir);
                    if (ms.pdf > 0 && c > 0) {
                        throughput = throughput * ((((albedo * ms.bsdf) * c) / ms.pdf));
                        if (russian_prob != 1.0F) throughput = throughput / russian_prob;
                    }
                    else {
                        flags |= F_TERMINATED;
                    }
                    bool nee_final = false;
                    if constexpr (REGEN) {
                        bool cont = false;
                        if (!(flags & F_TERMINATED)) {
                            pdfb = ms.pdf;
                            flags = (m.attrib & ATN_MTRL_ATTR_SINGULAR) ? (flags | F_SINGULAR) : (flags & ~F_SINGULAR);
                            cont = bounce + 1 < fp.max_depth;
                            nee_final = !cont;
                        }
                        if (cont) {
                            const f3 no = ray_offset(rec.p, ray_along_normal);
                            const f3 nd = normalize(next_dir);
                            pb.ray_o[slot] = make_float4(no.x, no.y, no.z, pdfb);
                            pb.ray_d[slot] = make_float4(nd.x, nd.y, nd.z, __uint_as_float(regen_pack_d(flags, (uint32_t)(bounce + 1), rg_sample, rg_item)));
                            pb.thr[slot] = make_float4(throughput.x, throughput.y, throughput.z, __uint_as_float(regen_pack_t(smp.dim, rg_item)));
                            push_next = true;
                        }
                        else {
                            rg_end = regen_end(nee_final);
                            contrib_changed = false;
                            push_next = rg_end == 1u;
                        }
                        rg_stored = true; thr_stored = true; wrote_ray = true;
                    }
                    else {
                    pb.thr[slot] = make_float4(throughput.x, throughput.y, throughput.z, __uint_as_float(smp.dim));
                    thr_stored = true;
                    if (!(flags & F_TERMINATED)) {
                        pdfb = ms.pdf;
                        flags = (m.attrib & ATN_MTRL_ATTR_SINGULAR) ? (flags | F_SINGULAR) : (flags & ~F_SINGULAR);
                        if (SVGF) {
                            const bool last_spec = m.id >= 0 && m.id < sc.n_materials && sc.materials[m.id].type == ATN_MTRL_SPECULAR;
                            flags = last_spec ? (flags | F_LAST_SPECULAR) : (flags & ~F_LAST_SPECULAR);
                        }
                        const f3 no = ray_offset(rec.p, ray_along_normal);
                        const f3 nd = normalize(next_dir);
                        pb.ray_o[slot] = make_float4(no.x, no.y, no.z, pdfb);
                        pb.ray_d[slot] = make_float4(nd.x, nd.y, nd.z, __uint_as_float(flags));
                        wrote_ray = true;
                        push_next = (bounce + 1 < fp.max_depth);
                    }
                    }
                    if (nee && !(flags & F_TERMINATED)) {
                        Cmj sl; sl.idx = smp.idx; sl.dim = nee_dim + 1u; sl.scramble = smp.scramble;
                        const int32_t li = nee_light;
                        const float lightSelectPdf = sc.inv_n_lights;
                        LightSample ls;
                        sample_light(ls, sc.lights[li], sc, rec.p, orienting_normal, sl, &hp);
                        push_shadow = radiance_nee_then<MS>(sc, ray_dir, orienting_normal, m, rec.u, rec.v, lightSelectPdf, ls, mtrl_slot, pre_r, nullptr,
                                                            [&](const f3& radiance) {
                            const float lbits = __uint_as_float((uint32_t)li | ((m.attrib & kAttrStencilAlways) ? kShadowStencilFlag : 0u)
                                                                | (nee_final ? kShadowFinalFlag : 0u));
                            const f3 lightcontrib = (thr_in * radiance) * albedo;
                            pb.sh_c[slot] = make_float4(lightcontrib.x, lightcontrib.y, lightcontrib.z, lbits);
                            const f3 dirToLight = normalize(ls.dir);
                            const float distToLight = length(ls.pos - rec.p);
                            const f3 so = ray_offset(rec.p, orienting_normal);
                            pb.sh_o[slot] = make_float4(so.x, so.y, so.z, distToLight);
                            pb.sh_d[slot] = make_float4(dirToLight.x, dirToLight.y, dirToLight.z, lbits);
                        }, &hp);
                    }
                }
            }
            if constexpr (REGEN) {
                if (!rg_stored) {
                    rg_end = regen_end(false);
                    contrib_changed = false;
                    push_next = rg_end == 1u;
                    thr_stored = true;
                }
            }
            else if (!push_next && !wrote_ray) {
                pb.ray_d[slot] = make_float4(rd4.x, rd4.y, rd4.z, __uint_as_float(flags));
            }
            if (!thr_stored) pb.thr[slot] = make_float4(throughput.x, throughput.y, throughput.z, __uint_as_float(smp.dim));
            if (contrib_changed) {
                const f3 contrib = mk3(pb.contrib[slot]) + contrib_add;
                pb.contrib[slot] = make_float4(contrib.x, contrib.y, contrib.z, 0.0F);
            }
            if constexpr (REGEN) rg_need_bits = rg_end & 12u;
        }
        if constexpr (REGEN) {
            if (valid) order[0].oflag[order[0].inv[e]] = (uint8_t)((push_next ? 1u : 0u) | (push_shadow ? 2u : 0u) | rg_need_bits);
        }
        else push_bits |= (push_next ? 1u << k : 0u) | (push_shadow ? 0x10000u << k : 0u);
      }
#if ATN_SHADE_PARTITION
      auto entry_of = [&](int k) { return part.perm[(uint32_t)k * 256u + threadIdx.x]; };
#else
      auto entry_of = [&](int k) { return q[chunk + (uint32_t)k * 256u + threadIdx.x]; };
#endif
      if constexpr (REGEN) {
          __syncthreads();
          {
              const uint32_t tid2 = here_v(threadIdx.x);
              const uint32_t lane2 = tid2 & 63u, wave2 = tid2 >> 6;
              uint32_t tot = 0;
#pragma unroll 1
              for (int k = 0; k < items; k++) {
                  const uint32_t jl = (uint32_t)k * 256u + threadIdx.x;
                  const bool need = jl < n_valid && (order[0].oflag[jl] & 4u) != 0u;
                  tot += (uint32_t)__popcll(__ballot(need));
              }
              if (lane2 == 0u) sh.wave_total[0][wave2] = tot;
              __syncthreads();
              if (threadIdx.x == 0u) {
                  const uint32_t a = sh.wave_total[0][0] + sh.wave_total[0][1] + sh.wave_total[0][2] + sh.wave_total[0][3];
                  sh.base[0] = a ? atomicAdd(pb.next_item, a) : 0u;
              }
              __syncthreads();
              uint32_t off = sh.base[0];
              for (uint32_t w = 0; w < wave2; w++) off += sh.wave_total[0][w];
#pragma unroll 1
              for (int k = 0; k < items; k++) {
                  const uint32_t jl = (uint32_t)k * 256u + threadIdx.x;
                  uint32_t f = jl < n_valid ? (uint32_t)order[0].oflag[jl] : 0u;
                  const bool need = (f & 4u) != 0u;
                  const unsigned long long m = __ballot(need);
                  if (need) {
                      const uint32_t item = off + bits_below_lane(m);
                      const uint32_t slot2 = q[chunk + jl];
                      const uint32_t pend_flag = (f & 8u) ? F_PENDING : 0u;
                      if (item < fp.n_items) {
                          const RegenState st = regen_primary_state(pb, fp, cam, item, 0u, pend_flag);
                          pb.ray_o[slot2] = st.o; pb.ray_d[slot2] = st.d; pb.thr[slot2] = st.t;
                          pb.contrib[slot2] = make_float4(0.0F, 0.0F, 0.0F, 0.0F);
                          f |= 1u;
                      }
                      else {
                          pb.ray_d[slot2] = make_float4(0.0F, 0.0F, 0.0F, __uint_as_float(pend_flag));
                      }
                  }
                  off += (uint32_t)__popcll(m);
                  push_bits |= ((f & 1u) << k) | (((f >> 1) & 1u) << (16 + k));
              }
              __syncthreads();
          }
          auto entry_in_order = [&](int k) { return q[chunk + (uint32_t)k * 256u + threadIdx.x]; };
          const uint32_t c = chunk / chunk_size;
          block_append2<decltype(entry_in_order), true>(sh, pb.q_regions + chunk, &pb.region_counts[2u * c], push_bits & 0xffffu,
                                                        pb.sh_regions + chunk, &pb.region_counts[2u * c + 1u], push_bits >> 16, entry_in_order);
          if (threadIdx.x < 2u) { const uint32_t v = pb.region_counts[2u * c + threadIdx.x]; if (v) atomicAdd(&pb.group_counts[2u * (c / kRegenGroup) + threadIdx.x], v); }
      }
      else
      block_append2(sh, qn, &pb.q_count[bounce_arg + 1], push_bits & 0xffffu, pb.shadow_q, &pb.sh_count[bounce_arg], push_bits >> 16, entry_of);
    }
#if !ATN_SHADE_PARTITION
    if (pb.stats) wave_add_stat(&pb.stats[2], nhits);
#endif
}

template <bool SVGF, int MS>
__global__ void ATN_SHADE_ATTR __launch_bounds__(256) k_shade(PathBuffers pb, DevScene sc, FrameParams fp, atn_camera_param cam, int32_t bounce, SvgfShade sv)
{
    shade_body<SVGF, MS>(pb, sc, fp, cam, bounce, sv);
}
template <bool SVGF, int MS, int WAVES>
__global__ void __attribute__((amdgpu_waves_per_eu(WAVES, WAVES))) __launch_bounds__(256) k_shade_wn(PathBuffers pb, DevScene sc, FrameParams fp, atn_camera_param cam, int32_t bounce, SvgfShade sv)
{
    shade_body<SVGF, MS>(pb, sc, fp, cam, bounce, sv);
}


template <bool ALPHA, bool REGEN = false>
struct ShadowJob {
    PathBuffers pb;
    DevScene sc;
    float t_min;
    ATN_DEV void fetch(uint32_t j, float4& a, float4& b, float& stop_t) const { fetch_slot(pb.shadow_q[j], a, b, stop_t); }
    ATN_DEV void fetch_slot(uint32_t slot, float4& a, float4& b, float& stop_t) const
    {
        const float4 so = pb.sh_o[slot], sd = pb.sh_d[slot];
        const f3 dir = normalize(mk3(sd));
        const uint32_t lbits = __float_as_uint(sd.w);
        const atn_light_param* lp = &sc.lights[lbits & 0xffffffu];
        const bool has_obj = lp->type == ATN_LIGHT_AREA && lp->arealight_objid >= 0;
        const bool near_only = (lp->attrib & ATN_LIGHT_ATTR_SINGULAR) && !(lp->attrib & ATN_LIGHT_ATTR_INFINITE);
        bool planar = false;
        if (has_obj && sc.planar_lights != 0) {
            const float4 pl = sc.light_plane[lbits & 0xffffffu];
            const float cos_l = fabsf(dot(mk3(pl), dir));
            const float big = fmaxf(fmaxf(fabsf(so.x), fabsf(so.y)), fabsf(so.z));
            const float off = 1.7320508F * fmaxf(big * (300.0F * 1.1920929e-7F), 1.0F / 65536.0F);
            planar = pl.w != 0.0F && cos_l >= 0.01F && off <= 5e-4F * so.w * cos_l;
        }
        stop_t = has_obj ? (planar ? so.w * 0.999F : -kInf) : (near_only ? so.w : kInf);
        if (ALPHA && sc.any_alpha && (sc.enable_alpha_blending || (lbits & kShadowStencilFlag))) stop_t = -kInf;
        a = make_float4(so.x, so.y, so.z, so.w - kEps);
        b = make_float4(dir.x, dir.y, dir.z, __uint_as_float(slot));
    }
    ATN_DEV void cost(uint32_t payload, uint32_t nodes, uint32_t tris) const
    {
        const uint32_t slot = payload & kShadowSlotMask;
        if (pb.cost) { atomicAdd(&pb.cost[2u * slot], nodes); atomicAdd(&pb.cost[2u * slot + 1u], tris); }
    }
    ATN_DEV bool finish(uint32_t payload, const Hit& h, bool isHit, float4& ra, float4& rb, float& rstop) const
    {
        const uint32_t slot = payload & kShadowSlotMask;
        const uint32_t lookups = (payload >> 27) & 15u;
        const float4 lc = pb.sh_c[slot];
        const uint32_t lbits = __float_as_uint(lc.w);
        const atn_light_param* lp = &sc.lights[lbits & 0xffffffu];
        const int32_t ltype = lp->type, lobj = lp->arealight_objid;
        const uint32_t lattr = lp->attrib;
        const int32_t lightobj = (ltype == ATN_LIGHT_AREA && lobj >= 0) ? lobj : -1;
        const bool same_obj = isHit ? h.objid == lightobj : (lookups == 0u || (payload & (1u << 26)) != 0u);
        bool visible;
        if (same_obj) visible = true;
        else if (lattr & ATN_LIGHT_ATTR_INFINITE) visible = !isHit;
        else if (lattr & ATN_LIGHT_ATTR_SINGULAR) visible = h.t > pb.sh_o[slot].w;
        else visible = false;
        if (ALPHA && sc.any_alpha && isHit) {
            const bool need_stencil = (lbits & kShadowStencilFlag) != 0u;
            const uint32_t max_lookups = (sc.enable_alpha_blending || need_stencil) ? 10u : 1u;
            if (visible || max_lookups > 1u) {
                const int32_t mid = triangle_mtrlid(sc, h.tri);
                const uint32_t mattr = mid >= 0 ? sc.materials[mid].attrib : 0u;
                bool ignore = need_stencil && (mattr & kAttrStencilStencil);
                f3 hit_p = mk3(0.0F), hit_n = mk3(0.0F, 1.0F, 0.0F);
                if (ignore || (mattr & kAttrMaybeAlpha)) {
                    HitRec rec;
                    evaluate_hit(rec, sc, h.objid, h.tri, h.a, h.b);
                    hit_p = rec.p; hit_n = rec.normal;
                    if (mattr & kAttrMaybeAlpha) {
                        const DevMaterial& hm = sc.materials[mid];
                        const float4 albedo = sample_texture(sc, hm.albedoMap, rec.u, rec.v, make_float4(1.0F, 1.0F, 1.0F, 1.0F));
                        if (albedo.w * hm.baseColor.w < 1.0F) ignore = true;
                    }
                }
                if (ignore) {
                    if (lookups + 1u >= max_lookups) return false;
                    const float distToLight = pb.sh_o[slot].w;
                    const f3 odir = normalize(mk3(pb.sh_d[slot]));
                    const bool is_same_facing = dot(hit_n, odir) > 0.0F;
                    const f3 on = is_same_facing ? hit_n : -hit_n;
                    const f3 o = ray_offset(hit_p, on);
                    const f3 d = normalize(odir);
                    ra = make_float4(o.x, o.y, o.z, distToLight - kEps);
                    rb = make_float4(d.x, d.y, d.z, __uint_as_float(slot | ((lookups + 1u) << 27) | (h.objid == lightobj ? (1u << 26) : 0u)));
                    rstop = -kInf;
                    return true;
                }
            }
        }
        if (visible) {
            float4* dst = pb.contrib;
            if constexpr (REGEN) { if (lbits & kShadowFinalFlag) dst = pb.pend; }
            const float4 c = dst[slot];
            dst[slot] = make_float4(c.x + lc.x, c.y + lc.y, c.z + lc.z, REGEN ? c.w : 0.0F);
        }
        return false;
    }
};

template <bool COUNT, bool REFILL>
__global__ void __launch_bounds__(kTraceBlock > 256 ? kTraceBlock : 256) k_trace_shadow(PathBuffers pb, DevScene sc, int32_t bounce)
{
    const uint32_t count = pb.sh_count[bounce];
    const ShadowJob<true> job{ pb, sc, kEps };
    TravCounters tc{};
    trace_dispatch<COUNT, REFILL>(sc, count, &pb.fetch_shadow[bounce], job, &tc);
    if (COUNT) {
        if (blockIdx.x == 0 && threadIdx.x == 0) atomicAdd(&pb.stats[1], (unsigned long long)count);
        wave_add_stat(&pb.stats[5], tc.nodes);
        wave_add_stat(&pb.stats[6], tc.tris);
    }
}

template <bool ALPHA, bool REGEN = false>
struct FusedJob {
    ShadowJob<ALPHA, REGEN> s;
    ClosestJob c;
    uint32_t n_shadow;
    float t_min;
    ATN_DEV void fetch(uint32_t j, float4& a, float4& b, float& stop_t) const
    {
        if (j < n_shadow) {
            s.fetch(j, a, b, stop_t);
            b.w = __uint_as_float(__float_as_uint(b.w) | 0x80000000u);
        }
        else {
            c.fetch(j - n_shadow, a, b, stop_t);
        }
    }
    ATN_DEV bool finish(uint32_t payload, const Hit& h, bool is_hit, float4& ra, float4& rb, float& rstop) const
    {
        if (payload & 0x80000000u) {
            const bool again = s.finish(payload & 0x7fffffffu, h, is_hit, ra, rb, rstop);
            if (again) rb.w = __uint_as_float(__float_as_uint(rb.w) | 0x80000000u);
            return again;
        }
        return c.finish(payload, h, is_hit, ra, rb, rstop);
    }
    ATN_DEV void cost(uint32_t payload, uint32_t nodes, uint32_t tris) const
    {
        if (payload & 0x80000000u) s.cost(payload & 0x7fffffffu, nodes, tris); else c.cost(payload, nodes, tris);
    }
};

template <bool REFILL, bool ALPHA, bool LDSN = false, bool REGEN = false>
__global__ void ATN_TRACE_ATTR __launch_bounds__(kTraceBlock > 256 ? kTraceBlock : 256) k_trace_fused(PathBuffers pb, DevScene sc, int32_t bs, int32_t bc, int32_t launch)
{
    const uint32_t n_shadow = bs >= 0 ? pb.sh_count[bs] : 0u;
    const uint32_t n_closest = bc >= 0 ? pb.q_count[bc] : 0u;
    const FusedJob<ALPHA, REGEN> job{ ShadowJob<ALPHA, REGEN>{ pb, sc, kEps }, ClosestJob{ pb, pb.queue[(bc >= 0 ? bc : 0) & 1], kEps }, n_shadow, kEps };
    TravCounters tc{};
    trace_dispatch<false, REFILL, FusedJob<ALPHA, REGEN>, LDSN>(sc, n_shadow + n_closest, &pb.fetch_closest[launch], job, &tc);
}

template <int MS>
__global__ void __launch_bounds__(256) k_regen_shade(PathBuffers pb, DevScene sc, FrameParams fp, atn_camera_param cam, int32_t stage, RegenOut ro)
{
    shade_body<false, MS, true>(pb, sc, fp, cam, stage, SvgfShade{}, ro);
}
template <int MS, int WAVES>
__global__ void __attribute__((amdgpu_waves_per_eu(WAVES, WAVES))) __launch_bounds__(256) k_regen_shade_wn(PathBuffers pb, DevScene sc, FrameParams fp, atn_camera_param cam, int32_t stage, RegenOut ro)
{
    shade_body<false, MS, true>(pb, sc, fp, cam, stage, SvgfShade{}, ro);
}

#if ATN_MAIN_TU
__global__ void __launch_bounds__(256) k_accumulate_sample(PathBuffers pb, FrameParams fp)
{
    const uint32_t slot = (uint32_t)fp.slot_begin + blockIdx.x * blockDim.x + threadIdx.x;
    if (slot >= (uint32_t)fp.slot_end) return;
    int32_t x, y;
    if (!slot_to_pixel(fp, slot, x, y)) return;
    if (fp.sample > 0 && pb.done[slot]) return;
    const float4 c = pb.contrib[slot];
    const bool invalid = isnan(c.x) || isinf(c.x) || isnan(c.y) || isinf(c.y) || isnan(c.z) || isinf(c.z)
        || c.x < 0 || c.y < 0 || c.z < 0;
    if (invalid) return;
    float4 a = pb.accum[slot];
    a.x += c.x; a.y += c.y; a.z += c.z; a.w += 1.0F;
    pb.accum[slot] = a;
    const uint32_t flags = __float_as_uint(pb.ray_d[slot].w);
    if (fp.break_on_terminate && (flags & F_TERMINATED)) pb.done[slot] = 1;
}
#endif

template <bool ONE_SAMPLE>
__global__ void __launch_bounds__(256) k_gather(PathBuffers pb, FrameParams fp, float4* film, float4* tile_out)
{
    const uint32_t slot = blockIdx.x * blockDim.x + threadIdx.x;
    if (slot >= (uint32_t)fp.n_slots) return;
    int32_t x, y;
    float4 out = make_float4(0, 0, 0, 0);
    if (slot_to_pixel(fp, slot, x, y)) {
        float4 a;
        if (ONE_SAMPLE) {
            const float4 c = pb.contrib[slot];
            const bool invalid = isnan(c.x) || isinf(c.x) || isnan(c.y) || isinf(c.y) || isnan(c.z) || isinf(c.z)
                || c.x < 0 || c.y < 0 || c.z < 0;
            a = invalid ? make_float4(0.0F, 0.0F, 0.0F, 0.0F) : make_float4(0.0F + c.x, 0.0F + c.y, 0.0F + c.z, 1.0F);
        }
        else {
            a = pb.accum[slot];
        }
        const float cnt = a.w;
        const float4 v = make_float4(a.x / cnt, a.y / cnt, a.z / cnt, 1.0F);
        const uint32_t idx = (uint32_t)(y * fp.width + x);
        if (fp.progressive) {
            const float4 cur = film[idx];
            const float n = (float)((int32_t)cur.w);
            const float d = n + 1;
            out = make_float4((n * cur.x + v.x) / d, (n * cur.y + v.y) / d, (n * cur.z + v.z) / d, n + 1);
        }
        else {
            out = v;
        }
        film[idx] = out;
    }
    if (tile_out) tile_out[slot] = out;
}

#if ATN_MAIN_TU
__global__ void __launch_bounds__(256) k_assemble_tiles(const float4* __restrict__ gathered, float4* film,
                                                        int32_t width, int32_t height, int32_t tiles_x, int32_t tiles_y,
                                                        int32_t world, int32_t slots_per_rank)
{
    const uint32_t g = blockIdx.x * blockDim.x + threadIdx.x;
    if (g >= (uint32_t)(world * slots_per_rank)) return;
    FrameParams fp{};
    fp.width = width; fp.height = height; fp.tiles_x = tiles_x; fp.tiles_y = tiles_y; fp.tiles_x_rcp = udiv_rcp((uint32_t)tiles_x);
    fp.world = world; fp.rank = (int32_t)(g / (uint32_t)slots_per_rank);
    const uint32_t slot = g % (uint32_t)slots_per_rank;
    int32_t x, y;
    if (slot_to_pixel(fp, slot, x, y)) film[y * width + x] = gathered[g];
// ... 199 lines not shown
```

### aten_amd/csrc/device/scene_dev.hpp

```cpp
#pragma once
#include "vec.hpp"
#include "../../../include/aten_layout.h"

namespace atn {

constexpr int32_t kLinkEnd = -1;
constexpr int32_t kLinkLeafBit = 1;
constexpr int32_t kLinkTlasBit = 2;
constexpr int32_t kLinkTypeMask = 3;
constexpr int32_t kLinkNotInner = (int32_t)0x80000000u;
constexpr int32_t kLinkToLeaf = kLinkNotInner | kLinkLeafBit;
constexpr int32_t kLinkToTlas = kLinkNotInner | kLinkTlasBit;
constexpr uint32_t kLinkOffsetMask = 0x7ffffff0u;
constexpr int32_t kTlasIdentity = 1;
constexpr uint32_t kInnerBytes = 32;
constexpr uint32_t kTriLeafBytes = 48;
constexpr uint32_t kShadeTriQuads = 8;
constexpr int kMsCore = 0;
constexpr int kMsDisney = 1;
constexpr int kMsAnalytic = 2;
constexpr int kMsCarPaint = 3;
constexpr int kMsToon = 4;
constexpr uint32_t kLdsNodesMaxBytes = 32u * 1024u;

constexpr uint32_t kAttrIdealRefraction = 0x10000u;
constexpr uint32_t kAttrStencilAlways = 0x40000u;
constexpr uint32_t kAttrStencilStencil = 0x80000u;
constexpr uint32_t kAttrMaybeAlpha = 0x20000u;

struct DevMaterial {
    float4 baseColor;
    int32_t type;
    uint32_t attrib;
    int32_t id;
    int32_t albedoMap;
    int32_t normalMap;
    int32_t roughnessMap;
    float ior, roughness;
    float subsurface, metallic, specular, specularTint;
    float sheen, sheenTint, clearcoat, clearcoatGloss;
};
static_assert(sizeof(DevMaterial) == 80, "DevMaterial");

struct DevTexture {
    uint32_t offset;
    int32_t width, height;
    int32_t format;
};

struct DevScene {
    const float4* nodes;
    const atn_triangle_param* tris;
    const float4* shade_tris;
    const float4* vtx_pos;
    const float4* vtx_nml;
    const atn_object_param* objects;
    const float4* matrices;
    const DevMaterial* materials;
    const atn_toon_param* toon;
    const atn_light_param* npr_lights;
    const float* screen_shadow;
    int32_t n_npr_lights, ss_w, ss_h;
    int32_t enable_shadowray_base_stylized_shadow;
    const float4* carpaint;
    const atn_light_param* lights;
    const float4* texels;
    const uint32_t* texels8;
    const DevTexture* textures;
    int32_t n_lights;
    int32_t planar_lights;
    const float4* light_plane;
    float inv_n_lights;
    int32_t n_textures;
    int32_t n_materials;
    float bvh_hit_min;
    float bg_color[3];
    int32_t envmap_tex_idx;
    float avgIllum;
    float multiplyer;
    int32_t enable_env_map;
    int32_t any_alpha;
    int32_t enable_alpha_blending;
    int32_t material_set;
    int32_t root_link;
    float ibl_scene_radius;
    uint32_t node_bytes;
    uint32_t mtx_quads;
    int32_t ident_row;
    int32_t root_direct, root_objid, root_meshid, root_w2l, root_blas, root_flags;
    int32_t root_twin;
    float root_m[12];
    const float* ibl_cdf_v;
    const float* ibl_cdf_u;
    int32_t ibl_w, ibl_h;
    int32_t ibl_importance;
    int32_t tex_bilinear;
};

}
```

### aten_amd/csrc/host/scene_upload.hpp

```cpp
#pragma once
#include <cmath>
#include <cstring>
#include <string>
#include <vector>

#include "../device/scene_dev.hpp"
#include "anyhit_twin.hpp"

namespace atn {

struct HostSceneImage {
    std::vector<float4> nodes;
    uint64_t n_nodes = 0;
    std::vector<uint32_t> list_root;
    std::vector<int32_t> list_root_link;
    std::vector<uint32_t> list_bytes;
    std::vector<int32_t> list_twin_delta;
    struct TlasRef { uint32_t offset, list; };
    std::vector<TlasRef> tlas_refs;
    std::vector<uint32_t> list_tri_leaves, list_inner;
    std::vector<atn_triangle_param> tris;
    std::vector<float4> vtx_pos, vtx_nml;
    std::vector<atn_object_param> objects;
    std::vector<float4> matrices;
// ... 208 lines not shown
        if (s && o.light_id >= 0 && (uint32_t)o.light_id >= n_lights) { err = "object light id out of range"; return false; }
        if (s && o.type == ATN_OBJ_POLYGONS && o.triangle_num > 0
            && (o.triangle_id < 0 || (uint64_t)o.triangle_id + (uint64_t)o.triangle_num > n_tris)) { err = "object triangle range out of range"; return false; }
    }
    if (!s) return true;
    for (uint32_t i = 0; i < s->n_triangles; i++) {
        const atn_triangle_param& t = s->triangles[i];
        if (t.mtrlid >= 0 && (uint32_t)t.mtrlid >= s->n_materials) { err = "triangle material id out of range"; return false; }
        for (int v = 0; v < 3; v++)
            if (t.idx[v] < 0 || (uint32_t)t.idx[v] >= s->n_vertices) { err = "triangle vertex index out of range"; return false; }
    }
    for (uint32_t i = 0; i < s->n_lights; i++) {
        const atn_light_param& l = s->lights[i];
        if (l.arealight_objid >= 0 && (uint32_t)l.arealight_objid >= s->n_objects) { err = "light refers to an object id out of range"; return false; }
    }
    return true;
}

inline bool planar_area_light(const atn_scene_desc* s, const atn_light_param& l, float world_normal[3])
{
    const atn_mat4* l2w = nullptr;
    if (l.type != ATN_LIGHT_AREA || l.arealight_objid < 0 || (uint32_t)l.arealight_objid >= s->n_objects) return false;
    const atn_object_param* o = &s->objects[l.arealight_objid];
    if (o->type == ATN_OBJ_INSTANCE) {
        if (o->mtx_id >= 0) {
            if ((uint32_t)o->mtx_id + 1 >= s->n_matrices) return false;
            const atn_mat4& m = s->matrices[o->mtx_id + 1];
            for (int a = 0; a < 3; a++)
                for (int b = a; b < 3; b++) {
                    double d = 0;
                    for (int c = 0; c < 3; c++) d += (double)m.m[a][c] * (double)m.m[b][c];
                    if (std::fabs(d - (a == b ? 1.0 : 0.0)) > 1e-6) return false;
                }
            l2w = &s->matrices[o->mtx_id];
        }
        if (o->object_id < 0 || (uint32_t)o->object_id >= s->n_objects) return false;
        o = &s->objects[o->object_id];
    }
    if (o->type != ATN_OBJ_POLYGONS || o->triangle_num <= 0 || o->triangle_id < 0
        || (uint64_t)o->triangle_id + (uint64_t)o->triangle_num > s->n_triangles) return false;
    double p0[3] = { 0, 0, 0 }, n[3] = { 0, 0, 0 }, lo[3] = { 1e300, 1e300, 1e300 }, hi[3] = { -1e300, -1e300, -1e300 };
    bool have_plane = false;
    auto vtx = [&](int32_t i, double v[3]) { v[0] = s->vtx_pos[i].x; v[1] = s->vtx_pos[i].y; v[2] = s->vtx_pos[i].z; };
    for (int pass = 0; pass < 2; pass++) {
        for (int32_t t = o->triangle_id; t < o->triangle_id + o->triangle_num; t++) {
            const atn_triangle_param& tr = s->triangles[t];
            double v[3][3];
            for (int k = 0; k < 3; k++) {
                if (tr.idx[k] < 0 || (uint32_t)tr.idx[k] >= s->n_vertices) return false;
                vtx(tr.idx[k], v[k]);
            }
            if (pass == 0) {
                for (int k = 0; k < 3; k++) for (int a = 0; a < 3; a++) { lo[a] = std::min(lo[a], v[k][a]); hi[a] = std::max(hi[a], v[k][a]); }
                if (!have_plane) {
                    const double e1[3] = { v[1][0] - v[0][0], v[1][1] - v[0][1], v[1][2] - v[0][2] }, e2[3] = { v[2][0] - v[0][0], v[2][1] - v[0][1], v[2][2] - v[0][2] };
                    const double c[3] = { e1[1] * e2[2] - e1[2] * e2[1], e1[2] * e2[0] - e1[0] * e2[2], e1[0] * e2[1] - e1[1] * e2[0] };
                    const double len = std::sqrt(c[0] * c[0] + c[1] * c[1] + c[2] * c[2]);
                    if (len > 0) { for (int a = 0; a < 3; a++) { n[a] = c[a] / len; p0[a] = v[0][a]; } have_plane = true; }
                }
            }
            else {
                const double ext = std::sqrt((hi[0] - lo[0]) * (hi[0] - lo[0]) + (hi[1] - lo[1]) * (hi[1] - lo[1]) + (hi[2] - lo[2]) * (hi[2] - lo[2]));
                for (int k = 0; k < 3; k++) {
                    const double d = n[0] * (v[k][0] - p0[0]) + n[1] * (v[k][1] - p0[1]) + n[2] * (v[k][2] - p0[2]);
                    if (std::fabs(d) > 1e-9 * ext) return false;
                }
            }
        }
        if (!have_plane) return false;
    }
    double w[3] = { n[0], n[1], n[2] };
    if (l2w) {
        for (int a = 0; a < 3; a++) w[a] = (double)l2w->m[a][0] * n[0] + (double)l2w->m[a][1] * n[1] + (double)l2w->m[a][2] * n[2];
        const double len = std::sqrt(w[0] * w[0] + w[1] * w[1] + w[2] * w[2]);
        if (!(std::fabs(len - 1.0) <= 1e-5)) return false;
        for (int a = 0; a < 3; a++) w[a] /= len;
    }
    for (int a = 0; a < 3; a++) world_normal[a] = (float)w[a];
    return true;
}

constexpr double kTwinPays = 0.95;
constexpr uint64_t kTwinBudgetBytes = 512ull << 20;
inline bool build_host_image(HostSceneImage& img, const atn_scene_desc* s, std::string& err, int anyhit_twins = 0, int twin_dirs = 8,
                             int node_layout_top_levels = kLayoutTopLevels, bool planar_lights = true, uint64_t twin_budget_bytes = kTwinBudgetBytes)
{
    if (!s || s->n_bvh_lists == 0 || !s->bvh_lists) { err = "scene has no BVH lists"; return false; }
    const uint32_t nl = s->n_bvh_lists;
    std::string range_err;
    if (!validate_ranges(s->objects, s->n_objects, s->n_matrices, s, range_err)) { err = range_err; return false; }

    const uint32_t n_dir_wanted = twin_dirs == 8 ? 8u : 1u;
    uint64_t twin_bytes = 0, plain_bytes = 0;
    for (uint32_t k = 0; k < nl; k++) plain_bytes += (uint64_t)s->bvh_lists[k].count * 48u;
    std::vector<std::vector<ListLayout>> twin_lay(nl);
    std::vector<ListLayout> lay(nl);
    std::vector<std::vector<std::vector<atn_bvh_node>>> twin(nl);
    uint64_t total_nodes = 0;
    for (uint32_t k = 0; k < nl; k++) {
        if (!analyse_list(lay[k], s->bvh_lists[k].nodes, s->bvh_lists[k].count, k == 0, err)) return false;
        total_nodes += lay[k].order.size();
        if (k == 0 || !anyhit_twins || lay[k].order.size() != s->bvh_lists[k].count) continue;
        AnyhitTwin tw;
        if (!make_anyhit_twin(s->bvh_lists[k].nodes, s->bvh_lists[k].count, tw)) continue;
        if (anyhit_twins != 2 && !(tw.cost_twin <= kTwinPays * tw.cost_as_given)) continue;
        const uint64_t one = (uint64_t)s->bvh_lists[k].count * 48u;
        uint32_t n_dir = n_dir_wanted;
        auto fits = [&](uint32_t nd) {
            if (twin_bytes + one * nd > twin_budget_bytes) return false;
            return !(plain_bytes <= kLdsNodesMaxBytes && plain_bytes + twin_bytes + one * nd > kLdsNodesMaxBytes);
        };
        if (!fits(n_dir)) n_dir = 1u;
        if (!fits(n_dir)) continue;
        twin_bytes += one * n_dir;
        twin[k].resize(n_dir); twin_lay[k].resize(n_dir);
        bool ok = true;
        for (uint32_t g = 0; g < n_dir && ok; g++) {
            if (n_dir > 1) {
                const int sg[3] = { (g & 1u) ? 1 : -1, (g & 2u) ? 1 : -1, (g & 4u) ? 1 : -1 };
                ok = make_anyhit_twin(s->bvh_lists[k].nodes, s->bvh_lists[k].count, tw, sg);
            }
            std::string twin_err;
            ok = ok && analyse_list(twin_lay[k][g], tw.nodes.data(), (uint32_t)tw.nodes.size(), false, twin_err);
            twin[k][g].swap(tw.nodes);
        }
        if (!ok) { twin[k].clear(); twin_lay[k].clear(); }
    }
    uint64_t off = 0;
    img.list_root.assign(nl, 0);
    img.list_bytes.assign(nl, 0); img.list_tri_leaves.assign(nl, 0); img.list_inner.assign(nl, 0); img.list_twin_delta.assign(nl, 0);
    for (uint32_t kk = 1; kk <= nl; kk++) {
        const uint32_t k = kk % nl;
        img.list_root[k] = (uint32_t)off;
        for (uint32_t j = 0; j < lay[k].order.size(); j++) {
            if (lay[k].kind[j] == KIND_TRI) img.list_tri_leaves[k]++;
            else if (lay[k].kind[j] == KIND_INNER) img.list_inner[k]++;
        }
        assign_offsets(lay[k], off, k == 0 ? 0 : node_layout_top_levels);
        if (off >= (1ull << 31)) { err = "too many BVH nodes for 31-bit byte-offset links"; return false; }
        img.list_bytes[k] = (uint32_t)(off - img.list_root[k]);
        if (!twin[k].empty()) {
            if (twin_lay[k][0].kind[0] != lay[k].kind[0] || off + (uint64_t)img.list_bytes[k] * twin[k].size() >= (1ull << 31)) { twin[k].clear(); continue; }
            img.list_twin_delta[k] = (int32_t)(off - img.list_root[k]) | (twin[k].size() > 1 ? 1 : 0);
            for (size_t g = 0; g < twin[k].size(); g++)
                assign_offsets(twin_lay[k][g], off, node_layout_top_levels);
        }
    }
    if (off >= (1ull << 31)) { err = "too many BVH nodes for 31-bit byte-offset links"; return false; }
    img.nodes.assign((size_t)(off / 16), make_float4(0, 0, 0, 0));
    img.list_root_link.assign(nl, kLinkEnd);
    img.n_nodes = total_nodes;

    ListEmitCtx c;
    c.objects = s->objects; c.n_objects = s->n_objects; c.n_matrices = s->n_matrices; c.matrices = s->matrices;
    c.tris = s->triangles; c.vtx_pos = s->vtx_pos; c.n_triangles = s->n_triangles; c.n_vertices = s->n_vertices;
    c.n_lists = nl;
    uint64_t counts[3] = { 0, 0, 0 };
    img.tlas_refs.clear();
    for (uint32_t kk = 1; kk <= nl; kk++) {
        const uint32_t k = kk % nl;
        c.list_root_link = img.list_root_link.data();
        c.list_twin_delta = img.list_twin_delta.data();
        c.tlas_refs = &img.tlas_refs;
        int32_t root = kLinkEnd;
        if (!emit_list(reinterpret_cast<char*>(img.nodes.data()), lay[k], s->bvh_lists[k].nodes, c, root, counts, err)) return false;
        img.list_root_link[k] = root;
// ... 55 lines not shown
    }
    img.lights.assign(s->lights, s->lights + s->n_lights);
    img.light_plane.assign(s->n_lights ? s->n_lights : 1, make_float4(0, 0, 0, 0));
    for (uint32_t i = 0; i < s->n_lights; i++) {
        float wn[3];
        img.lights[i]._pad = 0;
        if (planar_lights && planar_area_light(s, s->lights[i], wn)) { img.light_plane[i] = make_float4(wn[0], wn[1], wn[2], 1.0F); img.lights[i]._pad = 1; }
    }
    img.params.planar_lights = planar_lights ? 1 : 0;
    img.textures.resize(s->n_textures);
    img.texels.clear(); img.texels8.clear();
    for (uint32_t i = 0; i < s->n_textures; i++) {
        const atn_texture_desc& t = s->textures[i];
        const size_t n = (size_t)t.width * t.height;
        int32_t fmt = 0;
        const size_t at8 = img.texels8.size();
        std::vector<uint32_t> packed(n);
        for (int32_t cand = 1; cand <= 2 && !fmt && n > 0; cand++) {
            auto decode = [cand](uint32_t k) { return cand == 1 ? (float)k / 255.0F : (float)k * (1.0F / 255); };
            auto code = [&](float v, uint32_t& k) {
                if (!(v >= 0.0F && v <= 1.0F)) return false;
                k = (uint32_t)(v * 255.0F + 0.5F);
                return k <= 255u && decode(k) == v;
            };
            bool ok = true;
            for (size_t j = 0; j < n && ok; j++) {
                uint32_t r = 0, g = 0, b = 0, a = 0;
                ok = code(t.texels[j].x, r) && code(t.texels[j].y, g) && code(t.texels[j].z, b) && code(t.texels[j].w, a);
                packed[j] = r | (g << 8) | (b << 16) | (a << 24);
            }
            if (ok) fmt = cand;
        }
        const bool unorm8 = fmt != 0;
        img.textures[i].width = t.width; img.textures[i].height = t.height;
        if (unorm8) {
            img.textures[i].offset = (uint32_t)at8; img.textures[i].format = fmt;
            img.texels8.insert(img.texels8.end(), packed.begin(), packed.end());
        }
        else {
            const size_t at = img.texels.size();
            img.textures[i].offset = (uint32_t)at; img.textures[i].format = 0;
            img.texels.resize(at + n);
            for (size_t j = 0; j < n; j++) img.texels[at + j] = make_float4(t.texels[j].x, t.texels[j].y, t.texels[j].z, t.texels[j].w);
        }
    }

    DevScene& p = img.params;
    p.root_link = img.list_root_link[0];
    fill_root_direct(p, img.nodes.data(), 0, s->matrices, s->n_matrices);
    p.n_lights = (int32_t)s->n_lights; p.inv_n_lights = s->n_lights ? 1.0f / (float)s->n_lights : 0.0f; p.n_textures = (int32_t)s->n_textures; p.n_materials = (int32_t)s->n_materials;
    p.bvh_hit_min = s->config.bvh_hit_min;
    p.bg_color[0] = s->config.bg.bg_color[0]; p.bg_color[1] = s->config.bg.bg_color[1]; p.bg_color[2] = s->config.bg.bg_color[2];
    p.envmap_tex_idx = s->config.bg.envmap_tex_idx;
    p.avgIllum = s->config.bg.avgIllum;
    p.multiplyer = s->config.bg.multiplyer;
    p.enable_env_map = s->config.bg.enable_env_map;
    p.any_alpha = 0;
    for (const DevMaterial& dm : img.materials) if (dm.attrib & (kAttrMaybeAlpha | kAttrStencilStencil)) p.any_alpha = 1;
    p.enable_alpha_blending = s->config.enable_alpha_blending ? 1 : 0;
    img.toon.assign((size_t)s->n_materials + 1, atn_toon_param{});
    for (uint32_t i = 0; i < s->n_materials; i++) {
        img.toon[i] = s->materials[i].toon;
        const int32_t t = s->materials[i].type;
        if (t == ATN_MTRL_TOON || t == ATN_MTRL_STYLIZED_BRDF) {
            const atn_toon_param& tp = img.toon[i];
            if (tp.target_light_idx >= 0 && (uint32_t)tp.target_light_idx >= s->n_npr_target_lights) { err = "toon material's target light index out of range"; return false; }
            if (tp.target_light_idx >= 0 && !s->npr_target_lights) { err = "null NPR target light array"; return false; }
        }
    }
    if (s->n_npr_target_lights && s->npr_target_lights) {
        img.npr_lights.assign(s->npr_target_lights, s->npr_target_lights + s->n_npr_target_lights);
        for (const atn_light_param& l : img.npr_lights)
            if (l.arealight_objid >= 0 && (uint32_t)l.arealight_objid >= s->n_objects) { err = "NPR target light refers to an object id out of range"; return false; }
    }
    p.n_npr_lights = (int32_t)img.npr_lights.size();
    p.enable_shadowray_base_stylized_shadow = s->enable_shadowray_base_stylized_shadow ? 1 : 0;
    p.ss_w = p.ss_h = 0;
    if (s->screen_space_texture.texels && s->screen_space_texture.width > 0 && s->screen_space_texture.height > 0) {
        p.ss_w = s->screen_space_texture.width; p.ss_h = s->screen_space_texture.height;
        const size_t n = (size_t)p.ss_w * p.ss_h;
        img.screen_shadow.resize(n);
        for (size_t i = 0; i < n; i++) img.screen_shadow[i] = s->screen_space_texture.texels[i].x;
    }
    p.material_set = kMsCore;
    for (const DevMaterial& dm : img.materials) {
        const int32_t t = dm.type;
        const bool core = t == ATN_MTRL_EMISSIVE || t == ATN_MTRL_DIFFUSE || t == ATN_MTRL_SPECULAR || t == ATN_MTRL_GGX;
        const int32_t need = (t == ATN_MTRL_TOON || t == ATN_MTRL_STYLIZED_BRDF) ? kMsToon
                           : t == ATN_MTRL_CARPAINT ? kMsCarPaint : t == ATN_MTRL_DISNEY ? kMsDisney : core ? kMsCore : kMsAnalytic;
        if (need > p.material_set) p.material_set = need;
    }
    {
        const float* mn = s->scene_bbox_min; const float* mx = s->scene_bbox_max;
        float radius = 10000.0F;
        const bool valid = !((mn[0] >= mx[0]) || (mn[1] >= mx[1]) || (mn[2] >= mx[2]));
        if (valid) {
            const float cx = (mn[0] + mx[0]) * 0.5F, cy = (mn[1] + mx[1]) * 0.5F, cz = (mn[2] + mx[2]) * 0.5F;
            const float dx = mx[0] - cx, dy = mx[1] - cy, dz = mx[2] - cz;
            const float r = std::sqrt((dx * dx + dy * dy) + dz * dz);
            const float theta = (3.14159265358979323846F * (30.0F) / 180.0F);
            radius = r / std::tan(theta / 2);
        }
        p.ibl_scene_radius = radius;
    }
    return true;
}

}
```

### aten_amd/renderer.py

```python
import ctypes as C

import numpy as np

from . import layout as L
from ._lib import Destination, K_NAMES, lib


class AtenAmdError(RuntimeError):
    pass


class PathTracing:
    def __init__(self, device=0):
        self._l = lib()
        self._ctx = C.c_void_p()
        rc = self._l.atn_create(C.byref(self._ctx), device)
        if rc != 0:
            raise AtenAmdError("atn_create failed (%d): no usable HIP device; libaten_amd has no CPU fallback" % rc)
        if self._l.atn_sizeof_scene_desc() != C.sizeof(L.SceneDesc):
            raise AtenAmdError("atn_scene_desc ABI mismatch")
        if self._l.atn_sizeof_destination() != C.sizeof(Destination):
            raise AtenAmdError("atn_destination ABI mismatch")
        self.width = self.height = 0
        self._skin_sizes = {}
# ... 70 lines not shown
        self._check(self._l.atn_skin_compute(self._ctx, skin, int(bool(is_restart)), mn.ctypes.data, mx.ctypes.data))
        return mn, mx

    def lbvh_rebuild_list_skinned(self, list_index, skin):
        self._check(self._l.atn_lbvh_rebuild_list_skinned(self._ctx, list_index, skin))

    def skin_buffer(self, skin, name):
        which = {"pos": 0, "nml": 1, "prev": 2, "bbox": 3, "area": 4}[name]
        nv, nt = self._skin_sizes.get(skin, (0, 0))
        out = np.zeros((max(nv, 1), 4), np.float32) if which < 3 else np.zeros(6 if which == 3 else max(nt, 1), np.float32)
        self._check(self._l.atn_skin_download(self._ctx, skin, which, out.ctypes.data))
        return out[:nv] if which < 3 else (out if which == 3 else out[:nt])

    def skin_scene_arrays(self, skin, n_vertices, n_triangles):
        out = dict(shade=np.zeros((n_triangles, 8, 4), np.float32), vtx_pos=np.zeros((n_vertices, 4), np.float32),
                   vtx_nml=np.zeros((n_vertices, 4), np.float32), triangles=np.zeros(n_triangles, L.TRIANGLE_PARAM))
        for which, k in ((5, "shade"), (6, "vtx_pos"), (7, "vtx_nml"), (8, "triangles")):
            self._check(self._l.atn_skin_download(self._ctx, skin, which, out[k].ctypes.data))
        return out

    def bvh_list_bytes(self, list_index):
        n = C.c_uint32(0)
        self._check(self._l.atn_skin_download_list(self._ctx, list_index, None, 0, C.byref(n)))
        out = np.zeros(n.value, np.uint8)
        self._check(self._l.atn_skin_download_list(self._ctx, list_index, out.ctypes.data, n.value, C.byref(n)))
        return out

    def skin_close(self, skin):
        self._check(self._l.atn_skin_destroy(self._ctx, skin))
        self._skin_sizes.pop(skin, None)

    def set_geometry_motion(self, on=True):
        self._check(self._l.atn_set_geometry_motion(self._ctx, int(bool(on))))

    def geometry_motion_stats(self):
        s = np.zeros(3, np.uint64)
        self._check(self._l.atn_geometry_motion_stats(self._ctx, s.ctypes.data))
        return dict(passes=int(s[0]), copies=int(s[1]), copied_float4=int(s[2]))

    def geometry_motion_matrices(self):
        a, b = np.zeros((4, 4), np.float32), np.zeros((4, 4), np.float32)
        self._check(self._l.atn_geometry_motion_matrices(self._ctx, a.ctypes.data, b.ctypes.data))
        return a, b

    def scene_device_arrays(self):
        p = [C.c_void_p() for _ in range(3)]
        self._check(self._l.atn_scene_device_arrays(self._ctx, C.byref(p[0]), C.byref(p[1]), C.byref(p[2])))
        return tuple(x.value for x in p)

    def updateCamera(self, cam):
        self._check(self._l.atn_update_camera(self._ctx, cam.ctypes.data))

    def initSampler(self, width, height, seed=0):
        self._check(self._l.atn_init_sampler(self._ctx, width, height, seed))

    def setRandom(self, seeds):
        seeds = np.ascontiguousarray(seeds, np.uint32)
        self._check(self._l.atn_set_random(self._ctx, seeds.ctypes.data, len(seeds)))

    def getRandom(self):
        out = np.zeros(self._l.atn_random_count(self._ctx), np.uint32)
        if len(out):
            self._check(self._l.atn_get_random(self._ctx, out.ctypes.data, len(out)))
        return out

    def setScreenShard(self, rank, world):
        self._check(self._l.atn_set_screen_shard(self._ctx, rank, world))

    def render(self, width, height, max_depth=5, rr_depth=3, spp=1, frame=0, progressive=True,
               break_on_terminate=True, download=True, count_stats=False, profile=False):
        d = Destination(width, height, max_depth, rr_depth, spp, frame, int(progressive),
                        int(break_on_terminate), int(count_stats), int(profile))
        out = np.empty((height, width, 4), np.float32) if download else None
        self._check(self._l.atn_render(self._ctx, C.byref(d), out.ctypes.data if download else None))
        self.width, self.height = width, height
        return out

    def set_upload_options(self, anyhit_twin=None, anyhit_twin_dirs=None, node_layout=None, planar_lights=None):
        v = lambda x: -1 if x is None else int(x)
        self._check(self._l.atn_set_upload_options(self._ctx, v(anyhit_twin), v(anyhit_twin_dirs), v(node_layout), v(planar_lights)))

    def set_shade_math(self, relaxed):
        self._check(self._l.atn_set_shade_math(self._ctx, int(relaxed)))

    def set_regeneration(self, on):
        self._check(self._l.atn_set_regeneration(self._ctx, int(on)))

    def render_burst(self, width, height, n_frames, max_depth=5, rr_depth=3, spp=1, frame=0, progressive=True,
                     break_on_terminate=True, download=True, profile=False):
        d = Destination(width, height, max_depth, rr_depth, spp, frame, int(progressive), int(break_on_terminate), 0, int(profile))
        out = np.empty((height, width, 4), np.float32) if download else None
        self._check(self._l.atn_render_burst(self._ctx, C.byref(d), n_frames, out.ctypes.data if download else None))
        self.width, self.height = width, height
        return out

    def regen_stage_counts(self):
        n = C.c_uint32(0)
        self._check(self._l.atn_regen_stage_counts(self._ctx, None, None, 0, C.byref(n)))
        q = np.zeros(n.value, np.uint32); sh = np.zeros(n.value, np.uint32)
        if n.value:
            self._check(self._l.atn_regen_stage_counts(self._ctx, q.ctypes.data, sh.ctypes.data, n.value, C.byref(n)))
        return q, sh

    def set_path_batches(self, n):
        self._check(self._l.atn_set_path_batches(self._ctx, n))

    def set_frames_in_flight(self, n):
        self._check(self._l.atn_set_frames_in_flight(self._ctx, n))

    def side_stream_ptr(self):
        p = self._l.atn_side_stream(self._ctx)
        if not p:
            raise AtenAmdError("atn_side_stream failed")
        return p

    def bank_streams(self):
        sw, cc = C.c_int32(0), C.c_int32(0)
        self._check(self._l.atn_bank_streams(self._ctx, C.byref(sw), C.byref(cc)))
        self.side_stream_concurrent = bool(cc.value & 2)
        return sw.value, bool(cc.value & 1)

    def set_sampling_options(self, ibl_importance=False, tex_bilinear=False):
        self._check(self._l.atn_set_sampling_options(self._ctx, int(ibl_importance), int(tex_bilinear)))

    def sample_texture(self, texid, uv):
        uv = np.ascontiguousarray(uv, np.float32).reshape(-1, 2)
        out = np.zeros((len(uv), 4), np.float32)
        self._check(self._l.atn_sample_texture(self._ctx, texid, len(uv), uv.ctypes.data, out.ctypes.data))
        return out

    def reset(self):
        self._check(self._l.atn_reset(self._ctx))

    def synchronize(self):
        self._check(self._l.atn_synchronize(self._ctx))

    def film_device_ptr(self):
        return self._l.atn_film_device(self._ctx)

    def tile_device_ptr(self):
        return self._l.atn_tile_device(self._ctx)

    def tile_slots(self):
        return int(self._l.atn_tile_slots(self._ctx))

    def stream_ptr(self):
        return self._l.atn_stream(self._ctx)

    def assemble_tiles(self, gathered_dev_ptr, world, out_dev_ptr=None, stream_ptr=None):
        self._check(self._l.atn_assemble_tiles_on(self._ctx, gathered_dev_ptr, world, out_dev_ptr, stream_ptr))

    def download_film(self):
        out = np.empty((self.height, self.width, 4), np.float32)
        self._check(self._l.atn_download_film(self._ctx, out.ctypes.data))
        return out

    def upload_film(self, film):
        film = np.ascontiguousarray(film, np.float32)
        h, w = film.shape[:2]
        self._check(self._l.atn_upload_film(self._ctx, w, h, film.ctypes.data))
        self.width, self.height = w, h

    def path_cost(self):
        out = np.zeros((self.height, self.width, 2), np.uint32)
        self._check(self._l.atn_download_path_cost(self._ctx, out.ctypes.data))
        return out
# ... 477 lines not shown
```

### include/aten_amd.h

```cpp
#ifndef ATEN_AMD_H_
#define ATEN_AMD_H_

#include "aten_layout.h"

#ifdef __cplusplus
extern "C" {
#endif

typedef struct atn_ctx atn_ctx;

typedef enum atn_status {
    ATN_OK = 0,
    ATN_ERR_INVALID_ARG = -1,
    ATN_ERR_NO_DEVICE = -2,
    ATN_ERR_HIP = -3,
    ATN_ERR_NO_SCENE = -4,
    ATN_ERR_UNSUPPORTED = -5,
    ATN_ERR_OUT_OF_MEMORY = -6
} atn_status;

typedef struct atn_destination {
    int32_t width;
    int32_t height;
    int32_t maxDepth;
    int32_t russianRouletteDepth;
    int32_t sample;
    uint32_t frame;
    int32_t progressive;
    int32_t break_on_terminate;
    int32_t count_stats;
    int32_t profile;
} atn_destination;

int atn_create(atn_ctx** out, int device_ordinal);
void atn_destroy(atn_ctx* ctx);
const char* atn_last_error(atn_ctx* ctx);

int atn_upload_scene(atn_ctx* ctx, const atn_scene_desc* scene);

int atn_update_tlas(atn_ctx* ctx, const atn_object_param* objects, uint32_t n_objects,
                    const atn_mat4* matrices, uint32_t n_matrices,
                    const atn_bvh_node* top_nodes, uint32_t n_top_nodes);

int atn_set_upload_options(atn_ctx* ctx, int32_t anyhit_twin, int32_t anyhit_twin_dirs, int32_t node_layout, int32_t planar_lights);

int atn_update_camera(atn_ctx* ctx, const atn_camera_param* camera);



int atn_update_geometry(atn_ctx* ctx, const atn_vec4* vtx_pos, const atn_vec4* vtx_nml, uint32_t n_vertices, uint32_t vtx_offset,
                        const atn_triangle_param* triangles, uint32_t n_triangles, uint32_t tri_offset);
int atn_scene_device_arrays(atn_ctx* ctx, void** vtx_pos, void** vtx_nml, void** triangles);
int atn_lbvh_rebuild_list(atn_ctx* ctx, uint32_t list_index, uint32_t tri_offset, uint32_t n_triangles,
                          const float bbox_min[3], const float bbox_max[3]);
int atn_lbvh_build(atn_ctx* ctx, const atn_triangle_param* triangles, uint32_t n_triangles, int32_t tri_id_offset,
                   const float bbox_min[3], const float bbox_max[3], const atn_vec4* vtx_pos, uint32_t n_vertices, int32_t vtx_offset,
                   atn_bvh_node* out_nodes, uint32_t* out_sorted_codes, uint32_t* out_sorted_indices);

typedef uint32_t atn_skin;
int atn_skin_create(atn_ctx* ctx, const atn_skinning_vertex* vertices, uint32_t n_vertices, uint32_t vtx_offset,
                    uint32_t tri_offset, uint32_t n_triangles, uint32_t n_matrices, atn_skin* out_skin);
int atn_skin_update(atn_ctx* ctx, atn_skin skin, const atn_mat4* matrices, uint32_t n);
int atn_skin_compute(atn_ctx* ctx, atn_skin skin, int32_t is_restart, float bbox_min[3], float bbox_max[3]);
int atn_lbvh_rebuild_list_skinned(atn_ctx* ctx, uint32_t list_index, atn_skin skin);
int atn_skin_download(atn_ctx* ctx, atn_skin skin, int32_t which, void* out_host);
int atn_skin_download_list(atn_ctx* ctx, uint32_t list_index, void* out_host, uint32_t capacity_bytes, uint32_t* n_bytes);
int atn_skin_destroy(atn_ctx* ctx, atn_skin skin);

int atn_init_sampler(atn_ctx* ctx, int32_t width, int32_t height, int32_t seed);
int atn_set_random(atn_ctx* ctx, const uint32_t* seeds, uint32_t n);
int atn_get_random(atn_ctx* ctx, uint32_t* out_host, uint32_t n);
uint32_t atn_random_count(atn_ctx* ctx);

int atn_set_screen_shard(atn_ctx* ctx, int32_t rank, int32_t world);

int atn_render(atn_ctx* ctx, const atn_destination* dst, atn_vec4* out_host);

int atn_set_regeneration(atn_ctx* ctx, int32_t mode);
int32_t atn_get_regeneration(atn_ctx* ctx);
int atn_render_burst(atn_ctx* ctx, const atn_destination* dst, int32_t n_frames, atn_vec4* out_host);
int atn_regen_stage_counts(atn_ctx* ctx, uint32_t* closest, uint32_t* shadow, uint32_t capacity, uint32_t* n_stages);

int atn_set_shade_math(atn_ctx* ctx, int32_t mode);

int atn_reset(atn_ctx* ctx);

void* atn_film_device(atn_ctx* ctx);
void* atn_tile_device(atn_ctx* ctx);
uint32_t atn_anyhit_twins(atn_ctx* ctx);
uint32_t atn_planar_area_lights(atn_ctx* ctx);
uint32_t atn_tile_slots(atn_ctx* ctx);
void* atn_stream(atn_ctx* ctx);
int atn_synchronize(atn_ctx* ctx);

int atn_assemble_tiles(atn_ctx* ctx, const void* gathered_dev, int32_t world, void* film_dev_out);
int atn_assemble_tiles_on(atn_ctx* ctx, const void* gathered_dev, int32_t world, void* film_dev_out, void* hip_stream);
int atn_download_film(atn_ctx* ctx, atn_vec4* out_host);
int atn_upload_film(atn_ctx* ctx, int32_t width, int32_t height, const atn_vec4* film_host);

int atn_get_stats(atn_ctx* ctx, uint64_t out[8]);
int atn_download_path_cost(atn_ctx* ctx, uint32_t* out_host);

enum { ATN_K_GEN = 0, ATN_K_TRACE_CLOSEST = 1, ATN_K_SHADE = 2, ATN_K_TRACE_SHADOW = 3,
       ATN_K_ACCUM = 4, ATN_K_GATHER = 5,
       ATN_K_SVGF_PREPARE = 6, ATN_K_SVGF_TEMPORAL = 7, ATN_K_SVGF_VARIANCE = 8, ATN_K_SVGF_ATROUS = 9,
       ATN_K_TRACE_FUSED = 10,
       ATN_K_COUNT = 11 };
int atn_get_kernel_times(atn_ctx* ctx, float ms[ATN_K_COUNT], uint32_t launches[ATN_K_COUNT]);
int atn_reset_kernel_times(atn_ctx* ctx);

int atn_set_path_batches(atn_ctx* ctx, int32_t n);

int atn_set_frames_in_flight(atn_ctx* ctx, int32_t n);
int atn_bank_streams(atn_ctx* ctx, int32_t* swaps, int32_t* concurrent);
void* atn_side_stream(atn_ctx* ctx);

int atn_set_sampling_options(atn_ctx* ctx, int32_t ibl_importance, int32_t tex_bilinear);
int atn_sample_texture(atn_ctx* ctx, int32_t texid, uint32_t n, const float* uv_host, float* out_host);

typedef struct atn_mgpu atn_mgpu;
int atn_mgpu_create(atn_mgpu** out, const int32_t* devices, int32_t n_devices);
void atn_mgpu_destroy(atn_mgpu* mg);
const char* atn_mgpu_last_error(atn_mgpu* mg);
int32_t atn_mgpu_shard_count(atn_mgpu* mg);
int32_t atn_mgpu_shard_device(atn_mgpu* mg, int32_t shard);
int atn_mgpu_upload_scene(atn_mgpu* mg, const atn_scene_desc* scene);
int atn_mgpu_update_tlas(atn_mgpu* mg, const atn_object_param* objects, uint32_t n_objects,
                         const atn_mat4* matrices, uint32_t n_matrices,
                         const atn_bvh_node* top_nodes, uint32_t n_top_nodes);
int atn_mgpu_update_geometry(atn_mgpu* mg, const atn_vec4* vtx_pos, const atn_vec4* vtx_nml, uint32_t n_vertices, uint32_t vtx_offset,
                             const atn_triangle_param* triangles, uint32_t n_triangles, uint32_t tri_offset);
int atn_mgpu_lbvh_rebuild_list(atn_mgpu* mg, uint32_t list_index, uint32_t tri_offset, uint32_t n_triangles,
                               const float bbox_min[3], const float bbox_max[3]);
int atn_mgpu_update_camera(atn_mgpu* mg, const atn_camera_param* camera);
int atn_mgpu_init_sampler(atn_mgpu* mg, int32_t width, int32_t height, int32_t seed);
int atn_mgpu_set_random(atn_mgpu* mg, const uint32_t* seeds, uint32_t n);
int atn_mgpu_render(atn_mgpu* mg, const atn_destination* dst, atn_vec4* out_host);
int atn_mgpu_reset(atn_mgpu* mg);
int atn_mgpu_synchronize(atn_mgpu* mg);
void* atn_mgpu_film_device(atn_mgpu* mg);
int atn_mgpu_download_film(atn_mgpu* mg, atn_vec4* out_host);
int atn_mgpu_set_frames_in_flight(atn_mgpu* mg, int32_t n);
int atn_mgpu_set_regeneration(atn_mgpu* mg, int32_t mode);
int atn_mgpu_render_burst(atn_mgpu* mg, const atn_destination* dst, int32_t n_frames, atn_vec4* out_host);

int atn_svgf_render(atn_ctx* ctx, const atn_destination* dst, int32_t compute_motion,
                    atn_vec4* out_host, atn_vec4* stages_host);
int atn_svgf_set_motion_depth(atn_ctx* ctx, const atn_vec4* motion_depth, uint32_t n);
int atn_svgf_reset(atn_ctx* ctx);
int atn_svgf_set_atrous_iterations(atn_ctx* ctx, int32_t n);
int atn_svgf_set_dilate_temporal_weight(atn_ctx* ctx, int32_t on);
int atn_svgf_download(atn_ctx* ctx, int32_t which, atn_vec4* out_host);

int atn_set_geometry_motion(atn_ctx* ctx, int32_t on);
int atn_geometry_motion_stats(atn_ctx* ctx, uint64_t* out3);
int atn_geometry_motion_matrices(atn_ctx* ctx, float* w2c16, float* prev_w2c16);

int atn_restir_set_options(atn_ctx* ctx, int32_t mode, int32_t n_candidates);
int atn_restir_render(atn_ctx* ctx, const atn_destination* dst, int32_t compute_motion, atn_vec4* out_host);
int atn_restir_set_motion_depth(atn_ctx* ctx, const atn_vec4* motion_depth, uint32_t n);
int atn_restir_reset(atn_ctx* ctx);
int atn_restir_capture(atn_ctx* ctx, int32_t on);
int atn_restir_download(atn_ctx* ctx, int32_t which, void* out_host);

int atn_npr_render(atn_ctx* ctx, const atn_destination* dst, atn_vec4* out_host);
int atn_npr_reset(atn_ctx* ctx);
// ... 55 lines not shown
```

Baseline: 664.5 Mrays/s.

## Pre-roll Russian roulette at shade time and trace doomed rays as any-hit

The shade kernel now predicts the next bounce's Russian-roulette outcome by replaying the same CMJ sample draws, and marks rays that will be terminated with a doomed flag. The closest-hit trace stops a doomed ray at its first hit, since only whether it hits matters. The next shade pass partitions those rays into a third class and terminates them without doing material work. The goal is to avoid full closest-hit traversal and shading on paths the roulette will kill anyway; the cost is an extra classification pass and the need for the replayed RNG sequence to match exactly, and it only applies to qualifying material sets.

```diff
diff --git a/aten_amd/_lib.py b/aten_amd/_lib.py
--- a/aten_amd/_lib.py
+++ b/aten_amd/_lib.py
@@ -35,6 +35,7 @@
     "atn_mgpu_download_film",
     "atn_set_regeneration", "atn_get_regeneration", "atn_render_burst", "atn_regen_stage_counts",
     "atn_mgpu_set_regeneration", "atn_mgpu_render_burst", "atn_set_upload_options", "atn_libm_probe", "atn_set_shade_math",
+    "atn_set_rr_lookahead", "atn_rr_lookahead_active", "atn_rr_lookahead_stats",
 ]
 
 
@@ -88,6 +89,9 @@
         l.atn_set_upload_options.argtypes = [vp, C.c_int32, C.c_int32, C.c_int32, C.c_int32]
         l.atn_set_regeneration.argtypes = [vp, C.c_int32]
         l.atn_set_shade_math.argtypes = [vp, C.c_int32]
+        l.atn_set_rr_lookahead.argtypes = [vp, C.c_int32]
+        l.atn_rr_lookahead_active.argtypes = [vp]; l.atn_rr_lookahead_active.restype = C.c_int32
+        l.atn_rr_lookahead_stats.argtypes = [vp, vp]
         l.atn_get_regeneration.argtypes = [vp]; l.atn_get_regeneration.restype = C.c_int32
         l.atn_render_burst.argtypes = [vp, C.POINTER(Destination), C.c_int32, vp]
         l.atn_regen_stage_counts.argtypes = [vp, vp, vp, C.c_uint32, C.POINTER(C.c_uint32)]
diff --git a/aten_amd/csrc/aten_amd.hip b/aten_amd/csrc/aten_amd.hip
--- a/aten_amd/csrc/aten_amd.hip
+++ b/aten_amd/csrc/aten_amd.hip
@@ -99,6 +99,8 @@
     bool opt_node_layout = true, opt_planar_lights = true;
     bool env_atrous4 = true;
     int env_shade_waves = 0;
+    bool rr_lookahead_twin = true;
+    int rr_lookahead = 1;
     int env_flavour = -1;
 
     DevBuf<float4> nodes, vtx_pos, vtx_nml, matrices, texels, carpaint, shade_tris;
@@ -658,7 +660,7 @@
     std::vector<Span> spans;
     size_t ev_used = 0;
     hipStream_t prof_stream = nullptr;
-    uint64_t host_stats[8] = {};
+    uint64_t host_stats[16] = {};
 
     int fail(int code, const std::string& msg) { last_error = msg; return code; }
 
@@ -681,6 +683,8 @@
         if (const char* e = std::getenv("ATEN_AMD_SVGF_ATROUS4")) env_atrous4 = e[0] != '0';
         if (const char* e = std::getenv("ATEN_AMD_SHADE_WAVES")) { const int v = std::atoi(e); if (v == 4 || v == 5) env_shade_waves = v; }
         if (const char* e = std::getenv("ATEN_AMD_LDS_NODES")) env_lds_nodes = std::atoi(e) != 0;
+        if (const char* e = std::getenv("ATEN_AMD_RR_LOOKAHEAD")) rr_lookahead = std::max(0, std::min(2, std::atoi(e)));
+        if (const char* e = std::getenv("ATEN_AMD_RR_LOOKAHEAD_TWIN")) rr_lookahead_twin = std::atoi(e) != 0;
         if (const char* e = std::getenv("ATEN_AMD_ANYHIT_TWIN")) env_anyhit_twin = std::max(0, std::min(2, std::atoi(e)));
         if (const char* e = std::getenv("ATEN_AMD_ANYHIT_TWIN_DIRS")) env_anyhit_twin_dirs = std::atoi(e) == 1 ? 1 : 8;
         if (const char* e = std::getenv("ATEN_AMD_NODE_LAYOUT")) opt_node_layout = std::atoi(e) != 0;
@@ -1319,8 +1323,8 @@
             counters_depth = max_depth + 2;
         }
         if (!stats.p) {
-            ATN_HIP(stats.resize(8));
-            ATN_HIP(hipMemsetAsync(stats.p, 0, 64, stream));
+            ATN_HIP(stats.resize(16));
+            ATN_HIP(hipMemsetAsync(stats.p, 0, 128, stream));
         }
         return ATN_OK;
     }
@@ -1417,6 +1421,11 @@
         }, count, p.refill);
     }
 
+    bool rr_lookahead_frame(bool count) const
+    {
+        return rr_lookahead >= (count ? 2 : 1) && scene.rr_lookahead != 0 && !shade_math_relaxed && scene.material_set <= kMsAnalytic;
+    }
+
     template <bool SVGF>
     void launch_shade(const PassPlan& p, hipStream_t st, const PathBuffers& pb, const FrameParams& fp, int32_t b, const SvgfShade& sv)
     {
@@ -1424,8 +1433,15 @@
             relaxed_launch_shade(scene.material_set, p.shade_waves, p.shade_grid, st, pb, scene, fp, camera, b);
             return;
         }
+        const bool la = !SVGF && pb.doomed_bit != 0u && b >= fp.rr_depth;
         with_shade_flavour(scene.material_set, p.shade_waves, [&](auto k) {
             using K = decltype(k);
+            if constexpr (!SVGF && K::waves != 0) {
+                if (la) {
+                    hipLaunchKernelGGL((k_shade_wn<false, K::ms, K::waves, true>), dim3(p.shade_grid), dim3(256), 0, st, pb, scene, fp, camera, b, sv);
+                    return;
+                }
+            }
             if constexpr (K::waves == 0) hipLaunchKernelGGL((k_shade<SVGF, K::ms>), dim3(p.shade_grid), dim3(256), 0, st, pb, scene, fp, camera, b, sv);
             else hipLaunchKernelGGL((k_shade_wn<SVGF, K::ms, K::waves>), dim3(p.shade_grid), dim3(256), 0, st, pb, scene, fp, camera, b, sv);
         });
@@ -1488,6 +1504,8 @@
             hipStream_t st = nb > 1 ? bstream[k] : stream;
             if (nb > 1) ATN_HIP(hipStreamWaitEvent(st, ev_fork, 0));
             PathBuffers pb = buffers(count, k, begin);
+            pb.doomed_bit = (!SVGF && rr_lookahead_frame(count)) ? F_DOOMED : 0u;
+            pb.doomed_stop = rr_lookahead_twin ? kInf : 1.0e30F;
             fp.slot_begin = (int32_t)begin; fp.slot_end = (int32_t)end;
             const uint32_t n = end - begin;
             const PassPlan plan = plan_pass(SVGF ? PassKind::Svgf : PassKind::Serial, n);
@@ -1589,7 +1607,7 @@
         if (rc) return rc;
         FrameParams fp = frame_params(*d);
         if (count) {
-            ATN_HIP(hipMemsetAsync(stats.p, 0, 64, stream));
+            ATN_HIP(hipMemsetAsync(stats.p, 0, 128, stream));
             ATN_HIP(cost.resize((size_t)2 * n_slots));
             ATN_HIP(cost_film.resize((size_t)2 * d->width * d->height));
             ATN_HIP(hipMemsetAsync(cost.p, 0, (size_t)2 * n_slots * sizeof(uint32_t), stream));
@@ -1614,12 +1632,15 @@
 
         if (count) {
             hipLaunchKernelGGL(k_cost_to_pixels, dim3(g_all), dim3(256), 0, stream, fp, (const uint32_t*)cost.p, cost_film.p);
-            ATN_HIP(hipMemcpyAsync(host_stats, stats.p, 64, hipMemcpyDeviceToHost, stream));
+            ATN_HIP(hipMemcpyAsync(host_stats, stats.p, 128, hipMemcpyDeviceToHost, stream));
         }
         if (out_host) {
             ATN_HIP(hipMemcpyAsync(out_host, film.p, (size_t)d->width * d->height * sizeof(float4), hipMemcpyDeviceToHost, stream));
         }
         if (out_host || count) ATN_HIP(hipStreamSynchronize(stream));
+        if (count) {
+            host_stats[0] -= host_stats[8]; host_stats[3] -= host_stats[10]; host_stats[4] -= host_stats[11];
+        }
         return ATN_OK;
     }
 
@@ -3108,6 +3129,24 @@
     ctx->r.regen_mode = mode;
     return ATN_OK;
 }
+int atn_set_rr_lookahead(atn_ctx* ctx, int32_t mode)
+{
+    CTX_QUIET_OR_FAIL(ctx);
+    if (mode < 0 || mode > 2) return ctx->r.fail(ATN_ERR_INVALID_ARG, "roulette look-ahead mode out of range");
+    ctx->r.rr_lookahead = mode;
+    return ATN_OK;
+}
+int32_t atn_rr_lookahead_active(atn_ctx* ctx)
+{
+    return (ctx && ctx->r.has_scene && ctx->r.rr_lookahead_frame(false)) ? 1 : 0;
+}
+int atn_rr_lookahead_stats(atn_ctx* ctx, uint64_t out[4])
+{
+    CTX_OR_FAIL(ctx);
+    if (!out) return ctx->r.fail(ATN_ERR_INVALID_ARG, "null output");
+    for (int i = 0; i < 4; i++) out[i] = ctx->r.host_stats[8 + i];
+    return ATN_OK;
+}
 int atn_set_shade_math(atn_ctx* ctx, int32_t mode)
 {
     CTX_QUIET_OR_FAIL(ctx);
diff --git a/aten_amd/csrc/device/kernels.hpp b/aten_amd/csrc/device/kernels.hpp
--- a/aten_amd/csrc/device/kernels.hpp
+++ b/aten_amd/csrc/device/kernels.hpp
@@ -27,6 +27,7 @@
 constexpr uint32_t kRegenItemHiShift = 24u;
 constexpr uint32_t kRegenDimMask = 4095u, kRegenItemLoShift = 12u, kRegenItemLoMask = (1u << 20) - 1u;
 constexpr uint32_t kRegenMaxSpp = 1u << 11, kRegenMaxItems = 1u << 28;
+constexpr uint32_t F_DOOMED = 32u;
 constexpr uint32_t kShadowFinalFlag = 0x20000000u;
 
 struct PathBuffers {
@@ -56,6 +57,8 @@
     uint32_t* group_counts;
     const uint32_t* valid_list;
     uint32_t* next_item;
+    uint32_t doomed_bit;
+    float doomed_stop;
 };
 
 struct FrameParams {
@@ -362,15 +365,18 @@
     }
 }
 
-struct ClosestJob {
+template <bool DOOM>
+struct ClosestJobT {
     PathBuffers pb;
     const uint32_t* __restrict__ q;
     float t_min;
+    uint32_t doomed_bit;
+    float doomed_stop;
     ATN_DEV void fetch(uint32_t j, float4& a, float4& b, float& stop_t) const { fetch_slot(q[j], a, b, stop_t); }
     ATN_DEV void fetch_slot(uint32_t slot, float4& a, float4& b, float& stop_t) const
     {
         const float4 ro = pb.ray_o[slot], rd = pb.ray_d[slot];
-        stop_t = -kInf;
+        stop_t = (DOOM && (__float_as_uint(rd.w) & doomed_bit)) ? doomed_stop : -kInf;
         a = make_float4(ro.x, ro.y, ro.z, kInf);
         b = make_float4(rd.x, rd.y, rd.z, __uint_as_float(slot));
     }
@@ -382,14 +388,18 @@
     ATN_DEV void cost(uint32_t slot, uint32_t nodes, uint32_t tris) const
     {
         if (pb.cost) { atomicAdd(&pb.cost[2u * slot], nodes); atomicAdd(&pb.cost[2u * slot + 1u], tris); }
+        if (DOOM && doomed_bit && pb.stats && (__float_as_uint(pb.ray_d[slot].w) & doomed_bit)) {
+            atomicAdd(&pb.stats[8], 1ull); atomicAdd(&pb.stats[10], (unsigned long long)nodes); atomicAdd(&pb.stats[11], (unsigned long long)tris);
+        }
     }
 };
+using ClosestJob = ClosestJobT<false>;
 
 template <bool COUNT, bool REFILL>
 __global__ void __launch_bounds__(kTraceBlock > 256 ? kTraceBlock : 256) k_trace_closest(PathBuffers pb, DevScene sc, int32_t bounce)
 {
     const uint32_t count = pb.q_count[bounce];
-    const ClosestJob job{ pb, pb.queue[bounce & 1], kEps };
+    const ClosestJobT<COUNT> job{ pb, pb.queue[bounce & 1], kEps, pb.doomed_bit, pb.doomed_stop };
     TravCounters tc{};
     trace_dispatch<COUNT, REFILL>(sc, count, &pb.fetch_closest[bounce], job, &tc);
     if (COUNT) {
@@ -414,16 +424,19 @@
 #ifndef ATN_SHADE_PARTITION
 #define ATN_SHADE_PARTITION 1
 #endif
-struct ShadePartShared { uint32_t perm[kChunk]; uint32_t wcount[kChunkItems][4][2]; };
+template <int NC> struct ShadePartSharedT { uint32_t perm[kChunk]; uint32_t wcount[kChunkItems][4][NC]; };
+using ShadePartShared = ShadePartSharedT<2>;
 template <bool ON> struct ShadeOrderShared { uint16_t inv[ON ? kChunk : 1]; uint8_t oflag[ON ? kChunk : 1]; };
 
-template <bool SVGF, int MS, bool REGEN = false>
+template <bool SVGF, int MS, bool REGEN = false, bool LA = false>
 ATN_DEV void shade_body(const PathBuffers& pb, const DevScene& sc, const FrameParams& fp, const atn_camera_param& cam, int32_t bounce_arg, const SvgfShade& sv,
                         const RegenOut& ro = RegenOut{})
 {
+    static_assert(!LA || (!SVGF && !REGEN && ATN_SHADE_PARTITION), "the look-ahead is the serial path tracer's");
     __shared__ BlockAppendShared sh;
+    const bool la_ends = LA && bounce_arg > fp.rr_depth;
 #if ATN_SHADE_PARTITION
-    __shared__ ShadePartShared part;
+    __shared__ ShadePartSharedT<LA ? 3 : 2> part;
     __shared__ ShadeOrderShared<REGEN> order[1];
 #endif
     const uint32_t count = pb.q_count[bounce_arg];
@@ -439,38 +452,62 @@
       uint32_t push_bits = 0;
 #if ATN_SHADE_PARTITION
       const uint32_t n_valid = count - chunk < chunk_size ? count - chunk : chunk_size;
+      uint32_t doomed_lo = 0, doomed_hi = 0;
       {
           const uint32_t tid = here_v(threadIdx.x);
           const uint32_t lane = tid & 63u, wave = tid >> 6;
-          uint32_t hitmask = 0;
           __syncthreads();
+          constexpr uint32_t NC = LA ? 3u : 2u;
+          uint32_t cls_bits = 0;
 #pragma unroll 1
           for (int k = 0; k < items; k++) {
               const uint32_t j = chunk + (uint32_t)k * 256u + threadIdx.x;
-              const bool valid = j < count;
-              const bool hit = valid && __float_as_int(pb.isect[q[j]].x) >= 0;
-              if (hit) hitmask |= 1u << k;
-              const unsigned long long bh = __ballot(hit), bm = __ballot(valid && !hit);
-              if (lane == 0) { part.wcount[k][wave][0] = (uint32_t)__popcll(bh); part.wcount[k][wave][1] = (uint32_t)__popcll(bm); }
+              uint32_t cls = 3u;
+              if (j < count) {
+                  const uint32_t s = q[j];
+                  cls = __float_as_int(pb.isect[s].x) >= 0 ? 0u : NC - 1u;
+                  if constexpr (LA) { if (la_ends && cls == 0u && (__float_as_uint(pb.ray_d[s].w) & F_DOOMED)) cls = 1u; }
+              }
+              cls_bits |= cls << (2 * k);
+#pragma unroll
+              for (uint32_t c = 0; c < NC; c++) {
+                  const uint32_t n = (uint32_t)__popcll(__ballot(cls == c));
+                  if (lane == 0) part.wcount[k][wave][c] = n;
+              }
           }
-          if (pb.stats) wave_add_stat(&pb.stats[2], (uint32_t)__popc(hitmask));
+          if (pb.stats) {
+              uint32_t n0 = 0, n1 = 0;
+              for (int k = 0; k < items; k++) { const uint32_t c = (cls_bits >> (2 * k)) & 3u; n0 += c == 0u; n1 += c == 1u; }
+              wave_add_stat(&pb.stats[2], n0);
+              if constexpr (LA) wave_add_stat(&pb.stats[9], n1);
+          }
           __syncthreads();
-          uint32_t total_hits = 0;
-          for (int k = 0; k < items; k++) for (uint32_t w = 0; w < 4; w++) total_hits += part.wcount[k][w][0];
-          uint32_t before_h = 0, before_m = 0;
+          uint32_t base[NC];
+          base[0] = 0u;
+#pragma unroll
+          for (uint32_t c = 1; c < NC; c++) {
+              uint32_t t = 0;
+              for (int k = 0; k < items; k++) for (uint32_t w = 0; w < 4; w++) t += part.wcount[k][w][c - 1u];
+              base[c] = base[c - 1u] + t;
+          }
+          if constexpr (LA) { doomed_lo = base[1]; doomed_hi = base[2]; }
 #pragma unroll 1
           for (int k = 0; k < items; k++) {
               const uint32_t j = chunk + (uint32_t)k * 256u + threadIdx.x;
-              const bool valid = j < count;
-              const bool hit = (hitmask >> k) & 1u;
-              const unsigned long long bh = __ballot(hit), bm = __ballot(valid && !hit);
-              uint32_t bh_w = before_h, bm_w = before_m;
-              for (uint32_t w = 0; w < 4; w++) {
-                  if (w < wave) { bh_w += part.wcount[k][w][0]; bm_w += part.wcount[k][w][1]; }
-                  before_h += part.wcount[k][w][0]; before_m += part.wcount[k][w][1];
+              const uint32_t cls = (cls_bits >> (2 * k)) & 3u;
+              uint32_t pos = 0;
+#pragma unroll
+              for (uint32_t c = 0; c < NC; c++) {
+                  const unsigned long long bc = __ballot(cls == c);
+                  uint32_t mine = base[c];
+                  for (uint32_t w = 0; w < 4; w++) {
+                      const uint32_t n = part.wcount[k][w][c];
+                      if (w < wave) mine += n;
+                      base[c] += n;
+                  }
+                  if (cls == c) pos = mine + bits_below_lane(bc);
               }
-              if (valid) {
-                  const uint32_t pos = hit ? bh_w + bits_below_lane(bh) : total_hits + bm_w + bits_below_lane(bm);
+              if (cls != 3u) {
                   part.perm[pos] = q[j];
                   if constexpr (REGEN) order[0].inv[pos] = (uint16_t)(j - chunk);
               }
@@ -491,16 +528,28 @@
         uint32_t rg_need_bits = 0u;
         uint32_t slot = 0;
 
-        if (valid) {
+        bool live = valid;
 #if ATN_SHADE_PARTITION
-            slot = part.perm[e];
+        if (valid) slot = part.perm[e];
 #else
-            slot = q[j];
-#endif
+        if (valid) slot = q[j];
+#endif
+#if ATN_SHADE_PARTITION
+        if constexpr (LA) {
+            if (e >= doomed_lo && e < doomed_hi) {
+                const uint32_t f = __float_as_uint(pb.ray_d[slot].w);
+                pb.ray_d[slot].w = __uint_as_float((f & ~F_DOOMED) | F_HIT | F_TERMINATED);
+                live = false;
+            }
+        }
+#endif
+
+        if (live) {
             const float4 ro4 = pb.ray_o[slot], rd4 = pb.ray_d[slot];
             const f3 ray_org = mk3(ro4), ray_dir = mk3(rd4);
             float pdfb = ro4.w;
             uint32_t flags = __float_as_uint(rd4.w);
+            if constexpr (LA) flags &= ~F_DOOMED;
             uint32_t rg_sample = 0u, rg_item = 0u;
             int32_t bounce = bounce_arg;
             if constexpr (REGEN) {
@@ -745,8 +794,27 @@
                         }
                         const f3 no = ray_offset(rec.p, ray_along_normal);
                         const f3 nd = normalize(next_dir);
+                        uint32_t mark = 0u;
+                        if constexpr (LA) {
+                            if (bounce + 1 > fp.rr_depth && bounce + 1 < fp.max_depth) {
+                                Cmj la; la.idx = smp.idx; la.dim = smp.dim; la.scramble = smp.scramble;
+                                if (sc.n_lights > 0) {
+                                    int32_t pick = 0;
+                                    if (here(sc.n_lights) > 1) {
+                                        pick = (int32_t)(cmj_next(la) * (float)here(sc.n_lights));
+                                        pick = pick < sc.n_lights - 1 ? pick : sc.n_lights - 1;
+                                    }
+                                    else la.dim++;
+                                    la.dim += light_sample_draws(sc.lights[pick], sc);
+                                }
+                                if (dot(throughput, throughput) > 0) {
+                                    const float p = cmj_next(la);
+                                    if (p >= max3(throughput)) mark = F_DOOMED;
+                                }
+                            }
+                        }
                         pb.ray_o[slot] = make_float4(no.x, no.y, no.z, pdfb);
-                        pb.ray_d[slot] = make_float4(nd.x, nd.y, nd.z, __uint_as_float(flags));
+                        pb.ray_d[slot] = make_float4(nd.x, nd.y, nd.z, __uint_as_float(flags | mark));
                         wrote_ray = true;
                         push_next = (bounce + 1 < fp.max_depth);
                     }
@@ -860,15 +928,15 @@
 #endif
 }
 
-template <bool SVGF, int MS>
+template <bool SVGF, int MS, bool LA = false>
 __global__ void ATN_SHADE_ATTR __launch_bounds__(256) k_shade(PathBuffers pb, DevScene sc, FrameParams fp, atn_camera_param cam, int32_t bounce, SvgfShade sv)
 {
-    shade_body<SVGF, MS>(pb, sc, fp, cam, bounce, sv);
-}
-template <bool SVGF, int MS, int WAVES>
+    shade_body<SVGF, MS, false, LA>(pb, sc, fp, cam, bounce, sv);
+}
+template <bool SVGF, int MS, int WAVES, bool LA = false>
 __global__ void __attribute__((amdgpu_waves_per_eu(WAVES, WAVES))) __launch_bounds__(256) k_shade_wn(PathBuffers pb, DevScene sc, FrameParams fp, atn_camera_param cam, int32_t bounce, SvgfShade sv)
 {
-    shade_body<SVGF, MS>(pb, sc, fp, cam, bounce, sv);
+    shade_body<SVGF, MS, false, LA>(pb, sc, fp, cam, bounce, sv);
 }
 
 
@@ -980,7 +1048,7 @@
 template <bool ALPHA, bool REGEN = false>
 struct FusedJob {
     ShadowJob<ALPHA, REGEN> s;
-    ClosestJob c;
+    ClosestJobT<!REGEN> c;
     uint32_t n_shadow;
     float t_min;
     ATN_DEV void fetch(uint32_t j, float4& a, float4& b, float& stop_t) const
@@ -1013,7 +1081,7 @@
 {
     const uint32_t n_shadow = bs >= 0 ? pb.sh_count[bs] : 0u;
     const uint32_t n_closest = bc >= 0 ? pb.q_count[bc] : 0u;
-    const FusedJob<ALPHA, REGEN> job{ ShadowJob<ALPHA, REGEN>{ pb, sc, kEps }, ClosestJob{ pb, pb.queue[(bc >= 0 ? bc : 0) & 1], kEps }, n_shadow, kEps };
+    const FusedJob<ALPHA, REGEN> job{ ShadowJob<ALPHA, REGEN>{ pb, sc, kEps }, ClosestJobT<!REGEN>{ pb, pb.queue[(bc >= 0 ? bc : 0) & 1], kEps, REGEN ? 0u : pb.doomed_bit, pb.doomed_stop }, n_shadow, kEps };
     TravCounters tc{};
     trace_dispatch<false, REFILL, FusedJob<ALPHA, REGEN>, LDSN>(sc, n_shadow + n_closest, &pb.fetch_closest[launch], job, &tc);
 }
diff --git a/aten_amd/csrc/device/scene_dev.hpp b/aten_amd/csrc/device/scene_dev.hpp
--- a/aten_amd/csrc/device/scene_dev.hpp
+++ b/aten_amd/csrc/device/scene_dev.hpp
@@ -95,6 +95,7 @@
     int32_t ibl_w, ibl_h;
     int32_t ibl_importance;
     int32_t tex_bilinear;
+    int32_t rr_lookahead;
 };
 
 }
diff --git a/aten_amd/csrc/host/scene_upload.hpp b/aten_amd/csrc/host/scene_upload.hpp
--- a/aten_amd/csrc/host/scene_upload.hpp
+++ b/aten_amd/csrc/host/scene_upload.hpp
@@ -314,6 +314,22 @@
 
 constexpr double kTwinPays = 0.95;
 constexpr uint64_t kTwinBudgetBytes = 512ull << 20;
+inline bool rr_lookahead_valid(const std::vector<DevMaterial>& materials)
+{
+    for (const DevMaterial& dm : materials) {
+        if (dm.attrib & (ATN_MTRL_ATTR_SINGULAR | ATN_MTRL_ATTR_TRANSLUCENT | ATN_MTRL_ATTR_EMISSIVE)) return false;
+        switch (dm.type) {
+        case ATN_MTRL_DIFFUSE: case ATN_MTRL_OREN_NAYAR: case ATN_MTRL_GGX: case ATN_MTRL_BECKMAN: case ATN_MTRL_VELVET:
+        case ATN_MTRL_RETROREFLECTIVE: case ATN_MTRL_DISNEY:
+        case ATN_MTRL_SPECULAR: case ATN_MTRL_REFRACTION: case ATN_MTRL_MICROFACET_REFRACTION:
+            break;
+        default:
+            return false;
+        }
+    }
+    return true;
+}
+
 inline bool build_host_image(HostSceneImage& img, const atn_scene_desc* s, std::string& err, int anyhit_twins = 0, int twin_dirs = 8,
                              int node_layout_top_levels = kLayoutTopLevels, bool planar_lights = true, uint64_t twin_budget_bytes = kTwinBudgetBytes)
 {
@@ -535,6 +551,7 @@
         img.screen_shadow.resize(n);
         for (size_t i = 0; i < n; i++) img.screen_shadow[i] = s->screen_space_texture.texels[i].x;
     }
+    p.rr_lookahead = rr_lookahead_valid(img.materials) ? 1 : 0;
     p.material_set = kMsCore;
     for (const DevMaterial& dm : img.materials) {
         const int32_t t = dm.type;
diff --git a/aten_amd/renderer.py b/aten_amd/renderer.py
--- a/aten_amd/renderer.py
+++ b/aten_amd/renderer.py
@@ -176,6 +176,17 @@
 
     def set_shade_math(self, relaxed):
         self._check(self._l.atn_set_shade_math(self._ctx, int(relaxed)))
+
+    def set_rr_lookahead(self, mode):
+        self._check(self._l.atn_set_rr_lookahead(self._ctx, int(mode)))
+
+    def rr_lookahead_active(self):
+        return bool(self._l.atn_rr_lookahead_active(self._ctx))
+
+    def rr_lookahead_stats(self):
+        s = np.zeros(4, np.uint64)
+        self._check(self._l.atn_rr_lookahead_stats(self._ctx, s.ctypes.data))
+        return dict(doomed_rays=int(s[0]), doomed_hits=int(s[1]), doomed_nodes=int(s[2]), doomed_tris=int(s[3]))
 
     def set_regeneration(self, on):
         self._check(self._l.atn_set_regeneration(self._ctx, int(on)))
diff --git a/include/aten_amd.h b/include/aten_amd.h
--- a/include/aten_amd.h
+++ b/include/aten_amd.h
@@ -82,6 +82,10 @@
 int atn_regen_stage_counts(atn_ctx* ctx, uint32_t* closest, uint32_t* shadow, uint32_t capacity, uint32_t* n_stages);
 
 int atn_set_shade_math(atn_ctx* ctx, int32_t mode);
+
+int atn_set_rr_lookahead(atn_ctx* ctx, int32_t mode);
+int32_t atn_rr_lookahead_active(atn_ctx* ctx);
+int atn_rr_lookahead_stats(atn_ctx* ctx, uint64_t out[4]);
 
 int atn_reset(atn_ctx* ctx);
 
```

Measured after the change: 699.3 Mrays/s (median of 6 runs). +5.2%, better.
